# rrwick/Autocycler

Measured on AMD Instinct MI355X. Metric: Mbp/sec through compress->unitig GFA (k=51), higher is better.
Workload: dtype u64

## Files before the change

autocycler_amd/_capi.py:

```python
import ctypes as C
import os
from pathlib import Path

_HERE = Path(__file__).resolve().parent
LIB_PATH = _HERE / "libautocycler_hip.so"


class HipLibraryMissing(RuntimeError):
    pass


class AutocyclerError(RuntimeError):
    """The text the reference would hand to quit_with_error (misc.rs:131-137)."""


class SeqView(C.Structure):
    _fields_ = [("fwd", C.c_char_p), ("length", C.c_uint32), ("id", C.c_uint16)]


class Position(C.Structure):
    _fields_ = [("pos", C.c_uint32), ("seq_id_and_strand", C.c_uint16)]


class Link(C.Structure):
# ... 164 lines not shown
    _fields_ = [("a", C.c_uint16), ("b", C.c_uint16), ("distance", C.c_double)]


class ClusterSummary(C.Structure):
    _fields_ = [("n_seqs", C.c_uint32), ("launches", C.c_uint32), ("rescans", C.c_uint64), ("compares", C.c_uint64), ("seconds", C.c_double)]

    def as_dict(self):
        return {n: getattr(self, n) for n, _ in self._fields_}


class ClusterQcRecord(C.Structure):
    _fields_ = [("node", C.c_uint16), ("container", C.c_uint16), ("size", C.c_uint32), ("assembly_count", C.c_uint32), ("fail", C.c_uint32),
                ("trusted", C.c_uint32), ("reserved", C.c_uint32), ("median_length", C.c_uint64), ("cluster_dist", C.c_double)]

    def as_dict(self):
        return {n: getattr(self, n) for n, _ in self._fields_ if n != "reserved"}


class ClusteringMetrics(C.Structure):
    _fields_ = [(n, C.c_uint32) for n in ("pass_cluster_count", "fail_cluster_count", "pass_contig_count", "fail_contig_count")] + \
               [(n, C.c_double) for n in ("pass_contig_fraction", "fail_contig_fraction", "cluster_balance_score", "cluster_tightness_score",
                                          "overall_clustering_score")]

    def as_dict(self):
        return {n: getattr(self, n) for n, _ in self._fields_}


class ClusterQcSummary(C.Structure):
    _fields_ = [(n, C.c_uint32) for n in ("n_seqs", "n_clusters", "rounds", "evaluations", "pair_batches", "launches", "readbacks", "reserved")] + \
               [(n, C.c_uint64) for n in ("alternatives", "node_pairs", "bytes_read_back")] + [("seconds", C.c_double), ("start_score", C.c_double)]

    def as_dict(self):
        return {n: getattr(self, n) for n, _ in self._fields_ if n != "reserved"}


class DepthGraph(C.Structure):
    _fields_ = [("seq_bytes", C.c_void_p), ("seq_begin", C.c_void_p), ("seq_len", C.c_void_p), ("n_unitigs", C.c_uint32),
                ("links", C.c_void_p), ("n_links", C.c_uint64)]


class DepthTotals(C.Structure):
    _fields_ = [("size", C.c_uint64)] + \
               [(n, C.c_uint64) for n in ("reads", "rejected_reads", "read_bases", "span_bases", "span_kmers", "hits", "distinct_kmers", "repeat_kmers",
                                          "table_slots")] + [("batches", C.c_uint32), ("launches", C.c_uint32), ("seconds_device", C.c_double)]

    def as_dict(self):
        return {n: getattr(self, n) for n, _ in self._fields_ if n != "size"}

ALLREDUCE_FN = C.CFUNCTYPE(C.c_int, C.c_void_p, C.c_void_p, C.c_uint64, C.c_int, C.c_int)

EXPORTS = ["ac_compress_build", "ac_compress_build_multi", "ac_multi_info_get", "ac_compress_build_device", "ac_pack_text", "ac_text_size", "ac_layout_text", "ac_kmer_count",
           "ac_stats_pre", "ac_stats_post", "ac_unitig_count", "ac_unitig", "ac_unitigs_bulk", "ac_paths_bulk", "ac_unitig_positions", "ac_links",
           "ac_path", "ac_timings_get", "ac_timings_get_sized", "ac_free", "ac_gfa_string", "ac_string_free", "ac_last_error",
           "ac_device_count", "ac_max_kmer", "ac_version", "ac_abi_version", "ac_set_host_side_device", "ac_source_hash", "ac_set_stage_timing", "ac_random_access_ceilings", "ac_random_access_ceilings_at", "ac_release_memory", "ac_end_repair_device", "ac_pairwise_distances", "ac_trim_paths", "ac_trim_path_slices", "ac_overlap_alignment", "ac_trim_max_unitigs", "ac_resolve_bridges", "ac_resolve_bridge_paths", "ac_path_distances", "ac_resolve_anchors", "ac_resolve_bridge_records", "ac_resolve_best_paths", "ac_resolve_distinct_paths", "ac_resolve_summary_get_sized", "ac_resolve_max_path", "ac_resolve_free", "ac_graph_components", "ac_components_from_links", "ac_components_records", "ac_components_of_unitig", "ac_components_members", "ac_components_unitig_flags", "ac_components_summary_get_sized", "ac_topology_name", "ac_components_free", "ac_graph_merge_plan", "ac_merge_plan_from_links", "ac_merge_chains", "ac_merge_members", "ac_merge_chain_of_unitig", "ac_merge_fixed_flags", "ac_merge_sequences", "ac_merge_links", "ac_merge_summary_get_sized", "ac_merge_free", "ac_graph_subsets", "ac_subsets_from_paths", "ac_subsets_records", "ac_subsets_unitigs", "ac_subsets_links", "ac_subsets_seqs", "ac_subsets_path_ends", "ac_subsets_dense", "ac_subsets_summary_get_sized", "ac_subsets_free", "ac_subsets_components", "ac_subsets_merge_plan", "ac_subsets_merged_paths", "ac_merged_paths_get", "ac_merged_paths_summary_get_sized", "ac_merged_paths_free", "ac_merge_finish", "ac_subsets_finish", "ac_finished_unitigs", "ac_finished_sequences", "ac_finished_new_of_old", "ac_finished_links", "ac_finished_paths", "ac_finished_summary_get_sized", "ac_finished_free", "ac_finished_gfa_string", "ac_finished_to_graph", "ac_apply_bridges", "ac_graph_resolve_apply", "ac_applied_unitigs", "ac_applied_bridge_of", "ac_applied_links", "ac_applied_bridge_sequences", "ac_applied_summary_get_sized", "ac_applied_free", "ac_applied_merge_plan", "ac_applied_finish", "ac_applied_gfa_string", "ac_resolve_graphs", "ac_clean_graph", "ac_graph_clean", "ac_cleaned_unitigs", "ac_cleaned_links", "ac_cleaned_summary_get_sized", "ac_cleaned_free", "ac_cleaned_merge_plan", "ac_cleaned_finish", "ac_cleaned_gfa_string", "ac_parse_tig_numbers", "ac_gfa_segment_types", "ac_clean_gfa", "ac_clean", "ac_trim_apply", "ac_graph_trim_apply", "ac_graph_trim", "ac_trimmed_records", "ac_trimmed_summary_get_sized", "ac_trimmed_free", "ac_trimmed_subsets", "ac_trimmed_finish", "ac_trimmed_yaml_string", "ac_trim_gfa", "ac_trim_dir", "ac_resolve_dir", "ac_cluster_tree_build", "ac_cluster_tree_from_distances", "ac_cluster_tree_from_nodes", "ac_cluster_nodes", "ac_cluster_merges", "ac_cluster_summary_get_sized", "ac_cluster_free", "ac_cluster_max_seqs", "ac_cluster_cut", "ac_cluster_assign", "ac_cluster_containment", "ac_cluster_newick", "ac_cluster_generate", "ac_cluster_qc_nodes", "ac_cluster_qc_clusters", "ac_cluster_qc_assignment", "ac_cluster_qc_records", "ac_cluster_qc_metrics", "ac_cluster_qc_trace", "ac_cluster_qc_summary_get_sized", "ac_cluster_qc_free", "ac_cluster_min_assemblies", "ac_cluster_seq_inputs", "ac_depth_begin", "ac_depth_begin_handles", "ac_depth_add_reads", "ac_depth_add_fastq", "ac_depth_totals_get", "ac_depth_kmer_counts", "ac_depth_finish", "ac_depth_free", "ac_selftest_primitives", "ac_selftest_scan", "ac_selftest_radix", "ac_selftest_segments", "ac_selftest_sort_cmp", "ac_selftest_scan_pool", "ac_selftest_wave", "ac_selftest_fills", "ac_selftest_fill_order", "ac_selftest_readback", "ac_selftest_scalar_chain", "ac_selftest_arena", "ac_selftest_launch", "ac_selftest_atomics", "ac_selftest_side_order", "ac_selftest_event_ring", "ac_verify_graph", "ac_verify_graph_device", "ac_graph_from_gfa", "ac_graph_kmer_size", "ac_graph_seq_info", "ac_decompress_seq", "ac_decompress_device", "ac_decompress",
           "ac_shard_begin", "ac_shard_fragment_sizes", "ac_shard_fragments_export", "ac_shard_build_union", "ac_shard_fragment_packed_words", "ac_shard_fragments_export_packed", "ac_shard_build_union_packed",
           "ac_shard_unitig_count", "ac_shard_table_capacity", "ac_shard_bitmap_words", "ac_shard_bitmap_export", "ac_shard_build_novel", "ac_shard_sib_words", "ac_shard_sib_export", "ac_shard_degrees",
           "ac_shard_degree_bytes", "ac_multi_info_get_sized", "ac_shard_links_export", "ac_shard_links_import",
           "ac_shard_query_count", "ac_shard_query_key_words", "ac_shard_queries_export", "ac_shard_answer", "ac_shard_walk", "ac_shard_queries_route", "ac_shard_walk_routed", "ac_shard_local_distinct", "ac_shard_set_distinct_upper_bound", "ac_shard_distinct_count", "ac_shard_degrees_export", "ac_shard_build_graph", "ac_gfa_string_parts", "ac_shard_reduce_export", "ac_shard_reduce_import", "ac_shard_finish", "ac_shard_set_allreduce", "ac_device_copy",
           "ac_shard_path_entries", "ac_shard_paths_export", "ac_shard_free", "ac_graph_set_paths", "ac_graph_seq_count", "ac_path_counts",
           "ac_seqs_load", "ac_seqs_from_raw", "ac_seqs_count", "ac_seqs_assembly_count", "ac_seqs_views", "ac_seqs_get",
           "ac_seqs_repair_seconds", "ac_seqs_metrics_yaml", "ac_seqs_free", "ac_compress_seqs", "ac_compress_dir", "ac_compress_dir_multi"]

_libs = {}


def load_library(path=None):
    path = Path(path) if path else LIB_PATH
    key = str(path)
    if key in _libs:
        return _libs[key]
    if not path.exists():
        raise HipLibraryMissing(f"{path} not found: build the HIP extension first (make -C autocycler_amd/csrc). "
                                "There is no CPU fallback.")
    try:
        if os.environ.get("AC_NO_TORCH"):
            raise ImportError
        import torch
    except ImportError:
        pass
    lib = C.CDLL(key)
    lib.ac_last_error.restype = C.c_char_p
    lib.ac_version.restype = C.c_char_p
    lib.ac_source_hash.restype = C.c_char_p
    lib.ac_kmer_count.restype = C.c_uint64
    lib.ac_kmer_count.argtypes = [C.c_void_p]
    lib.ac_stats_pre.restype = Stats
    lib.ac_stats_pre.argtypes = [C.c_void_p]
    lib.ac_stats_post.restype = Stats
    lib.ac_stats_post.argtypes = [C.c_void_p]
    lib.ac_unitig_count.restype = C.c_uint32
    lib.ac_unitig_count.argtypes = [C.c_void_p]
    lib.ac_max_kmer.restype = C.c_uint32
    lib.ac_text_size.restype = C.c_uint64
    lib.ac_free.argtypes = [C.c_void_p]
    lib.ac_string_free.argtypes = [C.c_void_p]
    lib.ac_unitig.argtypes = [C.c_void_p, C.c_uint32, C.POINTER(C.c_void_p), C.POINTER(C.c_uint32), C.POINTER(C.c_double)]
    lib.ac_unitig_positions.argtypes = [C.c_void_p, C.c_uint32, C.c_int, C.POINTER(C.POINTER(Position)), C.POINTER(C.c_uint32)]
    lib.ac_links.argtypes = [C.c_void_p, C.POINTER(C.POINTER(Link)), C.POINTER(C.c_uint64)]
    lib.ac_path.argtypes = [C.c_void_p, C.c_uint32, C.POINTER(C.POINTER(C.c_int32)), C.POINTER(C.c_uint32)]
    lib.ac_timings_get.argtypes = [C.c_void_p, C.POINTER(Timings)]
    lib.ac_shard_unitig_count.restype = C.c_uint32
    lib.ac_shard_unitig_count.argtypes = [C.c_void_p]
    lib.ac_shard_fragment_packed_words.restype = C.c_uint64
    lib.ac_shard_fragment_packed_words.argtypes = [C.c_void_p, C.c_uint64]
    lib.ac_shard_local_distinct.restype = C.c_uint64
    lib.ac_shard_local_distinct.argtypes = [C.c_void_p]
    lib.ac_shard_set_distinct_upper_bound.argtypes = [C.c_void_p, C.c_uint64]
# ... 136 lines not shown
    lib.ac_trimmed_summary_get_sized.argtypes = [C.c_void_p, C.POINTER(TrimmedSummary), C.c_size_t]
    lib.ac_trimmed_free.restype = None
    lib.ac_trimmed_free.argtypes = [C.c_void_p]
    lib.ac_trimmed_subsets.restype = C.c_void_p
    lib.ac_trimmed_subsets.argtypes = [C.c_void_p]
    lib.ac_trimmed_finish.argtypes = [C.c_void_p, C.c_void_p, C.c_void_p, C.c_int, C.POINTER(C.c_void_p)]
    lib.ac_trimmed_yaml_string.argtypes = [C.c_void_p, C.POINTER(C.c_void_p), C.POINTER(C.c_uint64)]
    lib.ac_trim_gfa.argtypes = [C.c_char_p, C.c_uint64, C.c_double, C.c_uint32, C.c_double, C.c_int, C.POINTER(C.c_void_p), C.POINTER(C.c_uint64), C.POINTER(C.c_void_p),
                                C.POINTER(TrimmedSummary)]
    lib.ac_trim_dir.argtypes = [C.c_char_p, C.c_double, C.c_uint32, C.c_double, C.c_int]
    lib.ac_resolve_dir.argtypes = [C.c_char_p, C.c_int]
    lib.ac_resolve_graphs.argtypes = [C.c_void_p, C.c_int, C.POINTER(C.c_void_p), C.POINTER(C.c_void_p), C.POINTER(C.c_void_p), C.POINTER(C.c_uint32)]
    lib.ac_cluster_tree_from_nodes.argtypes = [C.POINTER(ClusterNode), C.c_uint32, C.c_int32, C.POINTER(C.c_void_p)]
    lib.ac_cluster_nodes.argtypes = [C.c_void_p, C.POINTER(C.POINTER(ClusterNode)), C.POINTER(C.c_uint32), C.POINTER(C.c_int32)]
    lib.ac_cluster_merges.argtypes = [C.c_void_p, C.POINTER(C.POINTER(ClusterMerge)), C.POINTER(C.c_uint32)]
    lib.ac_cluster_summary_get_sized.restype = C.c_size_t
    lib.ac_cluster_summary_get_sized.argtypes = [C.c_void_p, C.POINTER(ClusterSummary), C.c_size_t]
    lib.ac_cluster_free.argtypes = [C.c_void_p]
    lib.ac_cluster_free.restype = None
    lib.ac_cluster_cut.argtypes = [C.c_void_p, C.c_double, C.c_void_p, C.c_uint32, C.c_void_p, C.POINTER(C.c_uint32)]
    lib.ac_cluster_assign.argtypes = [C.c_void_p, C.c_void_p, C.c_uint32, C.c_void_p, C.c_void_p, C.c_void_p, C.POINTER(C.c_uint32)]
    lib.ac_cluster_containment.argtypes = [C.c_void_p, C.c_uint32, C.c_void_p, C.c_uint32, C.c_double, C.c_void_p, C.c_void_p]
    lib.ac_cluster_newick.argtypes = [C.c_void_p, C.c_void_p, C.c_int, C.POINTER(C.c_void_p)]
    qc_in = [C.c_void_p, C.c_void_p, C.c_uint32, C.c_void_p, C.c_void_p, C.c_void_p, C.c_void_p, C.c_double, C.c_uint32]
    lib.ac_cluster_generate.argtypes = qc_in + [C.c_void_p, C.c_uint32, C.c_int, C.POINTER(C.c_void_p)]
    lib.ac_cluster_qc_nodes.argtypes = qc_in + [C.c_void_p, C.c_uint32, C.c_void_p, C.c_uint32, C.c_int, C.POINTER(C.c_void_p)]
    lib.ac_cluster_qc_clusters.argtypes = [C.c_void_p, C.POINTER(C.POINTER(C.c_uint16)), C.POINTER(C.c_uint32)]
    lib.ac_cluster_qc_assignment.argtypes = [C.c_void_p, C.POINTER(C.POINTER(C.c_uint16)), C.POINTER(C.c_uint32)]
    lib.ac_cluster_qc_records.argtypes = [C.c_void_p, C.POINTER(C.POINTER(ClusterQcRecord)), C.POINTER(C.c_uint32)]
    lib.ac_cluster_qc_metrics.argtypes = [C.c_void_p, C.POINTER(ClusteringMetrics)]
    lib.ac_cluster_qc_trace.argtypes = [C.c_void_p, C.POINTER(C.POINTER(C.c_uint32)), C.POINTER(C.c_uint32), C.POINTER(C.POINTER(C.c_double)),
                                        C.POINTER(C.POINTER(C.c_uint8)), C.POINTER(C.c_uint64)]
    lib.ac_cluster_qc_summary_get_sized.restype = C.c_size_t
    lib.ac_cluster_qc_summary_get_sized.argtypes = [C.c_void_p, C.POINTER(ClusterQcSummary), C.c_size_t]
    lib.ac_cluster_qc_free.argtypes = [C.c_void_p]
    lib.ac_cluster_qc_free.restype = None
    lib.ac_cluster_min_assemblies.argtypes = [C.c_void_p, C.c_uint32, C.POINTER(C.c_uint32)]
    lib.ac_cluster_seq_inputs.argtypes = [C.c_void_p, C.c_void_p, C.c_void_p, C.c_void_p, C.c_void_p, C.POINTER(C.c_uint32)]
    lib.ac_depth_begin.argtypes = [C.c_uint32, C.POINTER(DepthGraph), C.c_uint32, C.c_int, C.POINTER(C.c_void_p)]
    lib.ac_depth_begin_handles.argtypes = [C.c_uint32, C.POINTER(C.c_void_p), C.c_uint32, C.c_int, C.POINTER(C.c_void_p)]
    lib.ac_depth_add_reads.argtypes = [C.c_void_p, C.c_void_p, C.c_void_p, C.c_uint64]
    lib.ac_depth_add_fastq.argtypes = [C.c_void_p, C.c_char_p]
    lib.ac_depth_totals_get.argtypes = [C.c_void_p, C.POINTER(DepthTotals)]
    lib.ac_depth_kmer_counts.argtypes = [C.c_void_p, C.c_void_p, C.c_uint64, C.c_void_p, C.c_void_p, C.c_void_p]
    lib.ac_depth_finish.argtypes = [C.c_void_p, C.c_uint32, C.c_void_p, C.c_void_p]
    lib.ac_depth_free.argtypes = [C.c_void_p]
    lib.ac_depth_free.restype = None
    lib.ac_selftest_scan.argtypes = [C.c_int, C.c_int, C.c_void_p, C.c_uint64, C.c_int, C.c_int, C.c_int, C.c_void_p]
    lib.ac_selftest_radix.argtypes = [C.c_int, C.c_void_p, C.c_void_p, C.c_uint64, C.c_int, C.c_int, C.c_int, C.c_uint64, C.c_int, C.c_int, C.c_void_p, C.c_void_p]
    lib.ac_selftest_segments.argtypes = [C.c_int, C.c_int, C.c_void_p, C.c_void_p, C.c_uint64, C.c_uint64, C.c_int, C.c_void_p, C.POINTER(C.c_uint32)]
    lib.ac_selftest_sort_cmp.argtypes = [C.c_int, C.c_int, C.c_void_p, C.c_void_p, C.c_void_p, C.c_uint64, C.c_void_p, C.c_void_p, C.c_void_p]
    lib.ac_selftest_scan_pool.argtypes = [C.c_int, C.c_int, C.c_uint64, C.POINTER(C.c_uint64)]
    lib.ac_selftest_wave.argtypes = [C.c_int, C.c_int, C.c_void_p, C.c_void_p, C.c_void_p, C.c_void_p]
    lib.ac_selftest_fills.argtypes = [C.c_int, C.c_void_p, C.c_uint64, C.c_int, C.c_int, C.c_void_p, C.c_uint64, C.c_void_p]
    lib.ac_selftest_fill_order.argtypes = [C.c_int, C.c_uint64, C.c_int, C.c_uint64, C.c_uint64, C.c_int, C.c_uint64, C.c_int, C.c_uint64, C.c_int, C.c_void_p]
    lib.ac_selftest_readback.argtypes = [C.c_int, C.c_void_p, C.c_uint64, C.c_int, C.c_void_p, C.c_uint64, C.c_void_p, C.c_void_p]
    lib.ac_selftest_scalar_chain.argtypes = [C.c_int, C.c_void_p, C.c_uint64, C.c_void_p, C.c_void_p]
    lib.ac_selftest_arena.argtypes = [C.c_int, C.c_void_p, C.c_uint64, C.c_void_p, C.c_void_p, C.c_void_p, C.c_void_p]
    lib.ac_selftest_launch.argtypes = [C.c_int, C.c_int, C.c_uint64, C.c_void_p, C.c_void_p]
    lib.ac_selftest_atomics.argtypes = [C.c_int, C.c_int, C.c_uint64, C.c_uint64, C.c_void_p, C.c_void_p, C.c_uint32, C.c_void_p, C.c_void_p]
    lib.ac_selftest_side_order.argtypes = [C.c_int, C.c_int, C.c_int, C.c_uint32, C.c_uint64, C.c_void_p]
    lib.ac_selftest_event_ring.argtypes = [C.c_int, C.c_int, C.c_void_p, C.c_uint32, C.c_void_p]
    _libs[key] = lib
    return lib


def _check(lib, rc):
    if rc != 0:
        raise AutocyclerError(lib.ac_last_error().decode(errors="replace"))


class Graph:

    def __init__(self, lib, handle, n_seqs):
        self._lib, self._h, self.n_seqs = lib, handle, n_seqs

    def close(self):
        if self._h:
            self._lib.ac_free(self._h)
            self._h = None

    def __del__(self):
        try:
            self.close()
        except Exception:
            pass

    @property
    def kmer_count(self):
        return self._lib.ac_kmer_count(self._h)

    def _stats(self, fn):
        s = fn(self._h)
        return dict(unitigs=s.unitigs, links=s.links_one_way, total_length=s.total_length)

    @property
    def stats_pre(self):
        return self._stats(self._lib.ac_stats_pre)

    @property
    def stats_post(self):
        return self._stats(self._lib.ac_stats_post)

    @property
    def unitig_count(self):
        return self._lib.ac_unitig_count(self._h)

# ... 1476 lines not shown
    v = _np_in(vals, np.int32 if signed else np.uint32)
    ko, vo = np.empty_like(k), np.empty_like(v)
    _check(lib, lib.ac_selftest_radix(device, k.ctypes.data, v.ctypes.data, k.size, begin_bit, end_bit, int(signed), prep_n, prep_bits, int(prep_reuse),
                                      ko.ctypes.data, vo.ctypes.data))
    return ko, vo


def selftest_segments(op, seg, vals, n_segments, deferred_err=False, device=0, lib_path=None):
    import numpy as np
    lib = load_library(lib_path)
    s, v = _np_in(seg, np.uint32), _np_in(vals, np.uint64)
    out = np.empty(n_segments, dtype=np.uint64 if op == "min" else np.uint32)
    err = C.c_uint32()
    _check(lib, lib.ac_selftest_segments(device, {"min": 0, "argmin": 1}[op], s.ctypes.data, v.ctypes.data, s.size, n_segments, int(deferred_err), out.ctypes.data,
                                         C.byref(err)))
    return out, err.value


def selftest_sort_pairs_cmp(key_a, key_b, vals, device=0, lib_path=None):
    import numpy as np
    lib = load_library(lib_path)
    a, b, v = _np_in(key_a, np.uint64), _np_in(key_b, np.uint32), _np_in(vals, np.uint32)
    ao, bo, vo = np.empty_like(a), np.empty_like(b), np.empty_like(v)
    _check(lib, lib.ac_selftest_sort_cmp(device, 0, a.ctypes.data, b.ctypes.data, v.ctypes.data, a.size, ao.ctypes.data, bo.ctypes.data, vo.ctypes.data))
    return ao, bo, vo


def selftest_sort_indices_cmp(values, indices, device=0, lib_path=None):
    import numpy as np
    lib = load_library(lib_path)
    a, v = _np_in(values, np.uint64), _np_in(indices, np.uint32)
    vo = np.empty_like(v)
    _check(lib, lib.ac_selftest_sort_cmp(device, 1, a.ctypes.data, None, v.ctypes.data, v.size, None, None, vo.ctypes.data))
    return vo


def selftest_scan_pool(op="read", value=0, device=0, lib_path=None):
    lib = load_library(lib_path)
    out = (C.c_uint64 * 3)()
    _check(lib, lib.ac_selftest_scan_pool(device, {"read": 0, "advance": 1, "invalidate": 2}[op], value, out))
    return dict(cap=out[0], epoch=out[1], tickets=out[2])


def selftest_wave(program, in_u64, aux_i32, live_mask, out_init, device=0, lib_path=None):
    import numpy as np
    lib = load_library(lib_path)
    i, a, m = _np_in(in_u64, np.uint64), _np_in(aux_i32, np.int32), _np_in(live_mask, np.uint64)
    out = np.array(out_init, dtype=np.uint64)
    assert i.size == 256 and a.size == 256 and m.size == 4 and out.size == 256
    _check(lib, lib.ac_selftest_wave(device, program, i.ctypes.data, a.ctypes.data, m.ctypes.data, out.ctypes.data))
    return out


FILL_KINDS = {"all": 0, "from": 1, "first": 2, "side_stream": 3}
FILL_TRIGGERS = {"none": 0, "launch": 1, "launch_full": 2, "launch_wave_kernel": 3, "copy_h2d": 4, "copy_d2h": 5, "copy_d2d": 6, "stream_sync": 7,
                 "arena_rewind": 8, "after_main": 9, "main_event": 10}
READ_PATHS = {"copy_d2h": 0, "batch": 1, "batch_twice": 2, "to_host": 3, "read_scalar": 4, "side_stream": 5}
ARENA_OPS = {"alloc": 0, "mark": 1, "rewind": 2, "reset": 3, "reserve": 4, "release_all": 5, "set_grow": 6}
LAUNCHERS = {"launch": 0, "launch_full": 1, "launch_wave_kernel": 2, "sized": 3}
ATOMIC_OPS = {"add32": 0, "add64": 1, "min32": 2, "max32": 3, "min64": 4, "max64": 5, "or32": 6, "or64": 7, "xor64": 8, "fetch_or32": 9, "fetch_and32": 10,
              "cas32": 11, "cas64": 12, "load32": 13, "wave_alloc32": 14, "wave_add64": 15}
ATOMIC_THREADS = 64 * 256
LAUNCH_SLOTS = 1024


def selftest_fills(regions, trigger, pattern, drop_on_reset=False, device=0, lib_path=None):
    import numpy as np
    lib = load_library(lib_path)
    r = _np_in([(b, FILL_KINDS[k], a, v) for b, k, a, v in regions], np.uint64)
    span = np.array(pattern, dtype=np.uint8)
    launches = np.zeros(2, dtype=np.uint32)
    _check(lib, lib.ac_selftest_fills(device, r.ctypes.data, len(regions), FILL_TRIGGERS[trigger], int(drop_on_reset), span.ctypes.data, span.size, launches.ctypes.data))
    return span, (int(launches[0]), int(launches[1]))


def selftest_fill_order(n, byte1, w_lo, w_hi, w_val, from2, byte2, upto3, byte3, device=0, lib_path=None):
    import numpy as np
    lib = load_library(lib_path)
    out = np.empty(n, dtype=np.uint8)
    _check(lib, lib.ac_selftest_fill_order(device, n, byte1, w_lo, w_hi, w_val, from2, byte2, upto3, byte3, out.ctypes.data))
    return out


def selftest_readback(data, path, items, device=0, lib_path=None):
    import numpy as np
    lib = load_library(lib_path)
    d = _np_in(data, np.uint8)
    it = _np_in(items, np.uint64).reshape(-1, 2)
    out = np.full(int(it[:, 1].sum()) + 1, 0xA5, dtype=np.uint8)
    counters = np.zeros(2, dtype=np.uint32)
    _check(lib, lib.ac_selftest_readback(device, d.ctypes.data, d.size, READ_PATHS[path], it.ctypes.data, it.shape[0], out.ctypes.data, counters.ctypes.data))
    assert out[-1] == 0xA5
    ends = np.cumsum(it[:, 1]).astype(np.int64)
    return [out[e - int(b):e] for e, b in zip(ends, it[:, 1])], int(counters[0]), int(counters[1])


def selftest_scalar_chain(values, device=0, lib_path=None):
    import numpy as np
    lib = load_library(lib_path)
    v = _np_in(values, np.uint64)
    out = np.zeros_like(v)
    counters = np.zeros(2, dtype=np.uint32)
    _check(lib, lib.ac_selftest_scalar_chain(device, v.ctypes.data, v.size, out.ctypes.data, counters.ctypes.data))
    return out, int(counters[0]), int(counters[1])


# ... 108 lines not shown
```

autocycler_amd/csrc/capi_steps.cpp:

```cpp
#include <algorithm>
#include <cstddef>
#include <cstring>
#include <fstream>
#include <memory>
#include <string>

#include "capi_common.hpp"
#include "gfa_writer.hpp"
#include "graph_depth.hpp"

using namespace ac;
using namespace ac::abi;

extern "C" {

int ac_end_repair_device(uint32_t k, void* d_text, uint64_t n_text, const uint64_t* seq_off, const uint32_t* seq_len,
                         uint16_t* seq_d1, uint16_t* seq_d2, uint32_t n_seqs, int device, double* seconds, uint64_t* n_matches) {
    return guarded([&] {
        if (!d_text || n_seqs == 0) throw DeviceError("no sequences found in input assemblies");
        if (!seq_d1 || !seq_d2) throw DeviceError("null sequence table");
        {
            std::vector<uint16_t> zero(n_seqs, 0);
            validate_layout(k, n_text, seq_off, seq_len, zero.data(), zero.data(), n_seqs);
        }
// ... 1717 lines not shown
        DeviceCall call(device);
        VerifyReport r;
#ifdef AC_EMU
        verify_graph_device(g->g, text.data(), text.size(), off, len, &r);
#else
        void* d_text = nullptr;
        AC_HIP_CHECK(hipMalloc(&d_text, text.size() + 64));
        struct Free { void* p; ~Free() { (void)hipFree(p); } } fr{d_text};
        AC_HIP_CHECK(hipMemcpy(d_text, text.data(), text.size(), hipMemcpyHostToDevice));
        verify_graph_device(g->g, (const uint8_t*)d_text, text.size(), off, len, &r);
#endif
        fill_report(r, report);
    });
}

int ac_decompress_device(const ac_graph* g, int device, uint8_t* out, uint64_t out_bytes) {
    return guarded([&] {
        if (!g || !out) throw DeviceError("null pointer");
        if (!g->host_arrays || !g->host_paths) throw DeviceError("this rank kept no host arrays (sharded build, not the writing rank)");
        uint64_t need = 0;
        for (uint32_t l : g->seq_lens) need += l;
        if (out_bytes < need) throw DeviceError("ac_decompress_device: the buffer holds " + std::to_string(out_bytes) + " bytes, the sequences need " + std::to_string(need));
        DeviceCall call(device);
        decompress_device(g->g, g->seq_lens, out);
    });
}
int ac_selftest_primitives(int device, uint64_t n, uint64_t seed, int end_bit, int key_kind) {
    return guarded([&] {
        if (end_bit < 1 || end_bit > 64) throw DeviceError("end_bit out of range");
        DeviceCall call(device);
        primitives_selftest(n, seed, end_bit, key_kind);
    });
}
int ac_selftest_scan(int device, int kind, const void* in, uint64_t n, int in_place, int misalign_in, int misalign_out, void* out) {
    return guarded([&] { DeviceCall call(device); selftest_scan(kind, in, n, in_place != 0, misalign_in, misalign_out, out); });
}
int ac_selftest_radix(int device, const uint64_t* keys, const void* vals, uint64_t n, int begin_bit, int end_bit, int val_kind, uint64_t prep_n, int prep_bits,
                      int prep_reuse, uint64_t* keys_out, void* vals_out) {
    return guarded([&] { DeviceCall call(device); selftest_radix(keys, vals, n, begin_bit, end_bit, val_kind, prep_n, prep_bits, prep_reuse != 0, keys_out, vals_out); });
}
int ac_selftest_segments(int device, int op, const uint32_t* seg, const uint64_t* vals, uint64_t n, uint64_t n_segments, int deferred_err, void* out, uint32_t* err_out) {
    return guarded([&] { DeviceCall call(device); selftest_segments(op, seg, vals, n, n_segments, deferred_err != 0, out, err_out); });
}
int ac_selftest_sort_cmp(int device, int form, const uint64_t* key_a, const uint32_t* key_b, const uint32_t* vals, uint64_t n, uint64_t* key_a_out, uint32_t* key_b_out,
                         uint32_t* vals_out) {
    return guarded([&] { DeviceCall call(device); selftest_sort_cmp(form, key_a, key_b, vals, n, key_a_out, key_b_out, vals_out); });
}
int ac_selftest_scan_pool(int device, int op, uint64_t value, uint64_t* out) {
    return guarded([&] { DeviceCall call(device); selftest_scan_pool(op, value, out); });
}
int ac_selftest_wave(int device, int program, const uint64_t* in_u64, const int32_t* aux_i32, const uint64_t* live_mask, uint64_t* out_u64) {
    return guarded([&] { DeviceCall call(device); selftest_wave(program, in_u64, aux_i32, live_mask, out_u64); });
}
int ac_selftest_fills(int device, const uint64_t* regions, uint64_t n_regions, int trigger, int mode, uint8_t* span, uint64_t span_bytes, uint32_t* launches_out) {
    return guarded([&] { DeviceCall call(device); selftest_fills(regions, n_regions, trigger, mode, span, span_bytes, launches_out); });
}
int ac_selftest_fill_order(int device, uint64_t n, int byte1, uint64_t w_lo, uint64_t w_hi, int w_val, uint64_t from2, int byte2, uint64_t upto3, int byte3, uint8_t* out) {
    return guarded([&] { DeviceCall call(device); selftest_fill_order(n, byte1, w_lo, w_hi, w_val, from2, byte2, upto3, byte3, out); });
}
int ac_selftest_readback(int device, const uint8_t* data, uint64_t n_data, int path, const uint64_t* items, uint64_t n_items, uint8_t* out, uint32_t* counters_out) {
    return guarded([&] { DeviceCall call(device); selftest_readback(data, n_data, path, items, n_items, out, counters_out); });
}
int ac_selftest_scalar_chain(int device, const uint64_t* values, uint64_t n, uint64_t* out, uint32_t* counters_out) {
    return guarded([&] { DeviceCall call(device); selftest_scalar_chain(values, n, out, counters_out); });
}
int ac_selftest_arena(int device, const uint64_t* ops, uint64_t n_ops, uint64_t* totals_out, uint64_t* allocs_out, const uint8_t* live, uint64_t* wrong_out) {
    return guarded([&] { DeviceCall call(device); selftest_arena(ops, n_ops, totals_out, allocs_out, live, wrong_out); });
}
int ac_selftest_launch(int device, int which, uint64_t n, uint64_t* slots_out, uint32_t* info_out) {
    return guarded([&] { DeviceCall call(device); selftest_launch(which, n, slots_out, info_out); });
}
int ac_selftest_atomics(int device, int op, uint64_t init, uint64_t expected, const uint64_t* operand, const uint32_t* target, uint32_t n_words, uint64_t* words_out,
                        uint64_t* returns_out) {
    return guarded([&] { DeviceCall call(device); selftest_atomics(op, init, expected, operand, target, n_words, words_out, returns_out); });
}
int ac_selftest_side_order(int device, int mode, int which, uint32_t seed, uint64_t n_words, uint32_t* out_words) {
    return guarded([&] { DeviceCall call(device); selftest_side_order(mode, which, seed, n_words, out_words); });
}
int ac_selftest_event_ring(int device, int op, const uint8_t* kinds, uint32_t n_more, uint64_t* out) {
    return guarded([&] { DeviceCall call(device); selftest_event_ring(op, kinds, n_more, out); });
}

int ac_random_access_ceilings_at(int device, uint64_t table_slots, double* cas_gops, double* read_gops) {
    return guarded([&] {
        DeviceCall call(device);
        random_access_ceilings(cas_gops, read_gops, table_slots);
    });
}
int ac_random_access_ceilings(int device, double* cas_gops, double* read_gops) { return ac_random_access_ceilings_at(device, (uint64_t)1 << 24, cas_gops, read_gops); }

}
```

autocycler_amd/csrc/graph_build.hpp:

```cpp
#pragma once
#include <cstdint>
#include <functional>
#include <string>
#include <vector>

#include "graph_types.hpp"
#include "trim_host.hpp"
#include "resolve_host.hpp"
#include "components_host.hpp"
#include "merge_host.hpp"
#include "subset_host.hpp"
#include "trim_apply_host.hpp"
#include "finish_host.hpp"
#include "apply_host.hpp"
#include "clean_host.hpp"
#include "cluster_host.hpp"
#include "cluster_qc_host.hpp"

namespace ac {

struct SeqView {
    const uint8_t* fwd;
    uint32_t length;
};
// ... 125 lines not shown
void path_distance_batch(const PathPool& pool, const std::vector<PathPair>& pairs, const uint32_t* weights, std::vector<uint32_t>* dist,
                         ResolveDeviceStats* st);
uint32_t resolve_max_path();
struct ClusterDeviceStats { double seconds = 0; uint64_t rescans = 0, compares = 0; uint32_t launches = 0; };
void cluster_merges_device(const double* asym, uint32_t n, std::vector<ClusterRowMerge>* merges, ClusterDeviceStats* st);
void cluster_merges_graph_device(const FinalGraph& g, uint32_t n_seqs, double* asym_out, std::vector<ClusterRowMerge>* merges, ClusterDeviceStats* st);
uint32_t cluster_max_seqs();
struct ClusterQcDeviceStats {
    double seconds = 0;
    uint32_t launches = 0, readbacks = 0, evaluations = 0, pair_batches = 0;
    uint64_t alternatives = 0, pairs_counted = 0, bytes_read_back = 0;
};
void cluster_qc_device(const double* asym, uint32_t n, const uint32_t* dfs_tip, double cutoff, const std::function<void(const ClusterQcEvaluate&)>& body,
                       ClusterQcDeviceStats* st);
void components_device(uint32_t n_unitigs, const Link* links, uint64_t n_links, const uint32_t* unitig_len, const uint8_t* alive, const uint8_t* marked,
                       ComponentsResult* out);
struct MergePlanInput {
    uint32_t n_unitigs = 0; const Link* links = nullptr; uint64_t n_links = 0; const uint32_t* unitig_len = nullptr; const uint8_t* alive = nullptr;
    const uint8_t* seed_fixed = nullptr; const int32_t* path = nullptr; uint64_t n_path = 0;
    const uint8_t* seq_bytes = nullptr; const uint64_t* seq_begin = nullptr; uint64_t seq_total = 0;
};
void merge_plan_device(const MergePlanInput& in, MergeResult* out);
struct SubsetInput {
    uint32_t n_unitigs = 0; const Link* links = nullptr; uint64_t n_links = 0; const uint32_t* unitig_len = nullptr; const uint8_t* alive = nullptr;
    const int32_t* path = nullptr; const uint64_t* path_off = nullptr; uint32_t n_clusters = 0; const SubsetPlan* plan = nullptr;
};
void subsets_device(const SubsetInput& in, SubsetResult* out);
struct MergedPathsInput {
    uint32_t n_unitigs = 0; const uint32_t* unitig_len = nullptr; const int32_t* path = nullptr; const uint64_t* path_off = nullptr;
    const SubsetPlan* plan = nullptr; size_t kept_first = 0, kept_count = 0; const MergeResult* merge = nullptr;
};
void merged_paths_device(const MergedPathsInput& in, MergedPathsResult* out);
struct TrimApplyInput {
    uint32_t n_unitigs = 0; const Link* links = nullptr; uint64_t n_links = 0; const uint32_t* unitig_len = nullptr; const uint8_t* alive = nullptr;
    const int32_t* path = nullptr; const uint64_t* path_off = nullptr; double mad = 0;
};
void trim_apply_device(const TrimApplyInput& in, TrimApplyPlan* tp, SubsetPlan* plan, SubsetResult* out);
struct FinishInput {
    uint32_t n_unitigs = 0; const Link* links = nullptr; uint64_t n_links = 0; const uint32_t* unitig_len = nullptr; const uint8_t* alive = nullptr;
    const double* depth = nullptr; const uint8_t* type = nullptr; const uint8_t* seq_bytes = nullptr; const uint64_t* seq_begin = nullptr; uint64_t seq_total = 0;
    const MergeResult* plan = nullptr; const int32_t* path = nullptr; uint64_t n_path = 0; bool renumber = false; uint64_t unitigs_after = 0;
};
void merge_finish_device(const FinishInput& in, FinishResult* out);
void apply_bridges_device(const ApplyInput& in, const ApplyPlan& plan, ApplyResult* out);
void clean_device(const CleanInput& in, CleanResult* out);
void primitives_selftest(uint64_t n, uint64_t seed, int end_bit, int key_kind);
void selftest_scan(int kind, const void* in, uint64_t n, bool in_place, int misalign_in, int misalign_out, void* out);
void selftest_radix(const uint64_t* keys, const void* vals, uint64_t n, int begin_bit, int end_bit, int val_kind, uint64_t prep_n, int prep_bits, bool prep_reuse,
                    uint64_t* keys_out, void* vals_out);
void selftest_segments(int op, const uint32_t* seg, const uint64_t* vals, uint64_t n, uint64_t n_segments, bool deferred_err, void* out, uint32_t* err_out);
void selftest_sort_cmp(int form, const uint64_t* a, const uint32_t* b, const uint32_t* vals, uint64_t n, uint64_t* a_out, uint32_t* b_out, uint32_t* vals_out);
void selftest_scan_pool(int op, uint64_t value, uint64_t* out);
void selftest_wave(int program, const uint64_t* in_u64, const int32_t* aux_i32, const uint64_t* live_mask, uint64_t* out_u64);
void selftest_fills(const uint64_t* regions, uint64_t n_regions, int trigger, int mode, uint8_t* span, uint64_t span_bytes, uint32_t* launches_out);
void selftest_fill_order(uint64_t n, int byte1, uint64_t w_lo, uint64_t w_hi, int w_val, uint64_t from2, int byte2, uint64_t upto3, int byte3, uint8_t* out);
void selftest_readback(const uint8_t* data, uint64_t n_data, int path, const uint64_t* items, uint64_t n_items, uint8_t* out, uint32_t* counters_out);
void selftest_scalar_chain(const uint64_t* values, uint64_t n, uint64_t* out, uint32_t* counters_out);
void selftest_arena(const uint64_t* ops, uint64_t n_ops, uint64_t* totals_out, uint64_t* allocs_out, const uint8_t* live, uint64_t* wrong_out);
void selftest_launch(int which, uint64_t n, uint64_t* slots_out, uint32_t* info_out);
void selftest_atomics(int op, uint64_t init, uint64_t expected, const uint64_t* operand, const uint32_t* target, uint32_t n_words, uint64_t* words_out, uint64_t* returns_out);
void selftest_side_order(int mode, int which, uint32_t seed, uint64_t n_words, uint32_t* out_words);
void selftest_event_ring(int op, const uint8_t* kinds, uint32_t n_more, uint64_t* out);

void random_access_ceilings(double* cas_gops, double* read_gops, uint64_t table_slots = (uint64_t)1 << 24);

void device_warmup(int device, uint32_t k = 0, uint64_t text_bytes_estimate = 0);

void pack_text_host(const uint8_t* text, uint64_t n_text, uint64_t* bits, uint32_t* mask32, bool force_scalar);

void release_host_stager();

int max_supported_k();
void tuning_refresh();
int tuning_multi_transport();
bool tuning_multi_fragments_as_bytes();
bool tuning_multi_tail_replicated();
void set_stage_timing(bool on);
bool stage_timing();

}
```

autocycler_amd/csrc/graph_impl.hpp:

```cpp
#pragma once
#include "graph_build.hpp"

#include <chrono>
#include <cmath>
#include <map>
#include <string>
#include <algorithm>
#include <atomic>
#include <thread>
#include <functional>
#include <condition_variable>
#include <mutex>
#include <fcntl.h>
#include <unistd.h>
#if defined(__x86_64__)
#include <immintrin.h>
#endif

#include "device_rt.hpp"

namespace ac {

static double now_s() {
    return std::chrono::duration<double>(std::chrono::steady_clock::now().time_since_epoch()).count();
// ... 424 lines not shown
        seq_off.alloc(n_seqs); seq_len.alloc(n_seqs); seq_d1.alloc(n_seqs); seq_d2.alloc(n_seqs);
        copy_h2d(seq_off.ptr(), off.data(), (size_t)n_seqs * 8);
        copy_h2d(seq_len.ptr(), len.data(), (size_t)n_seqs * 4);
        copy_h2d(seq_d1.ptr(), d1.data(), (size_t)n_seqs * 2);
        copy_h2d(seq_d2.ptr(), d2.data(), (size_t)n_seqs * 2);
        has_flags = flags != nullptr;
        if (flags) { seq_flags.alloc(n_seqs); copy_h2d(seq_flags.ptr(), flags->data(), n_seqs); }
        n_bases = 0; any_dots = 0; n_dotted = 0; expected_nonbase = (u64)n_seqs + 1;
        for (u32 i = 0; i < n_seqs; i++) { n_bases += len[i]; if (d1[i] || d2[i]) { any_dots = 1; n_dotted++; } expected_nonbase += (u64)d1[i] + d2[i]; }
        stream_sync();
    }
    void alloc_table(u32 n) { n_seqs = n; h_off.clear(); h_len.clear(); seq_off.alloc(n); seq_len.alloc(n); seq_d1.alloc(n); seq_d2.alloc(n); seq_flags.alloc(n); has_flags = true; }
    void set_sums(u64 bases, u64 dotted, u64 dots) { n_bases = bases; n_dotted = dotted; any_dots = dotted ? 1 : 0; expected_nonbase = (u64)n_seqs + 1 + dots; }
    TextCtx ctx(int k) const { return TextCtx{bits.ptr(), mask.ptr(), n_text, k, seq_off.ptr(), seq_len.ptr(), seq_d1.ptr(), seq_d2.ptr(), n_seqs}; }
    bool packed = false;
    void pack_alloc(stream_t s = 0) {
        u64 n_bits_words = n_text / 32 + 24, n_mask_words = n_text / 64 + 12;
        bits.alloc(n_bits_words); mask.alloc(n_mask_words);
        const u64 groups = (n_text + 31) / 32;
        bits.fill_bytes_from(groups * 8, 0, s);
        mask.fill_bytes_from(groups * 4, 0xFF, s);
        if (check_alphabet) { pack_bad.alloc(2); pack_bad.fill_bytes(0xFF, s); }
    }
    void verify_alphabet(const u32* bad) const {
        if (!check_alphabet) return;
        if (bad[0] != 0xFFFFFFFFu) throw DeviceError("input sequence " + std::to_string(index_base + bad[0]) + " contains non-ACGT characters");
        const u64 found = (u64)(u32)(bad[1] + 1u);
        if (found != (expected_nonbase & 0xFFFFFFFFULL))
            throw DeviceError("the text does not match its sequence table: " + std::to_string(expected_nonbase) + " padding dots and separators expected, " +
                              std::to_string(found) + " non-ACGT characters found");
    }
    void pack() {
        if (packed) return;
        pack_alloc();
        launch((n_text + 31) / 32, PackFunctor{d_text, n_text, bits.ptr(), (u32*)mask.ptr(), 0, chk()});
        packed = true;
    }
};

struct GraphBuilder::Impl {
    u32 k = 0;
    DBuf<u8> text_owned;
    PackedText loc;
    PackedText uni;
    PackedText* G = &loc;
    BuildTimings* tm = nullptr;
    double t0 = 0, t_begin = 0;
    void lap(double* acc) { if (!g_stage_timing) return; stream_sync(); double t = now_s(); *acc += t - t0; t0 = t; }

    DBuf<u32> counters;
    DBuf<u64> slots; u64 cap = 0; u64 N = 0;
    DBuf<u64> bm; DBuf<u32> wprefix; DBuf<u64> npos;
    u32 U = 0;
    DBuf<u32> kinfo, head, scan, ustart, order, rank, ulen;
    DBuf<u64> ustartpos, useq_off; DBuf<u8> uorient;
    DBuf<int32_t> links; DBuf<u64> wlinks;
    DBuf<u32> depth, minpos_fwd, minpos_rev; DBuf<u64> path_off; DBuf<int32_t> ent_val; u64 n_ent = 0;
    DBuf<u64> wl_text; DBuf<u32> depth_u, minpos_fwd_u, minpos_rev_u, run_start, run_end;
    void walk_arrays();
    void walk_tables(bool filter);
    void walk_to_seed_order();
    bool walked_plain = false;
    DBuf<u8> fs0, fe0;
    u32 pos_cap_now = 0xFFFFFFFFu; bool exact_positions = false;
    bool host_remap_allowed = false;
    bool paths_in_seed_numbers = false;
    bool checked_sorts = false; DBuf<u32> sort_flags;
    bool deferred_sort_checks() const { return host_remap_allowed_build && !checked_sorts && sort_checks_deferrable(); }
    bool host_remap_allowed_build = false;
    DBuf<u8> maybe_dest; bool maybe_dest_valid = false;
    DBuf<u8> frag_text; DBuf<u64> frag_meta, frag_fpos, frag_boff; u64 frag_bytes = 0, n_frags = 0;
    u64 distinct_upper = 0;

    void begin(BuildTimings* t) {
        tm = t; t_begin = t0 = now_s();
        rt_counters() = RtCounters();
        host_remap_allowed = false;
        counters.alloc(8); counters.fill_bytes(0);
        sort_flags.alloc(2); sort_flags.fill_bytes(0);
    }
    void check_sizes(const PackedText& t) const {
        if (t.n_text >= POS_MASK) throw DeviceError("input too large for 40-bit text positions");
        if (t.n_seqs == 0 || t.n_text < (u64)k + 2) throw DeviceError("no sequences");
    }
    template <int W> void insert(const PackedText& t, u32 hint, DBuf<u64>* slots_out, u64* cap_out, u64* n_distinct_out, DBuf<u64>* bm_out, bool want_sib = false);
    DBuf<u64> sflags;
    DBuf<u64> runs; DBuf<u32> run_count; u64 run_rows = 0, run_rows_cap = 0;
    DBuf<u64> loc_bm; DBuf<u32> loc_wprefix; bool local_insert_of_shard = false;
    struct CopyPlan { bool ok = false; u64 R = 0, NW = 0, Rb = 0; DBuf<RunRec> rr; DBuf<u32> rseq; DBuf<u64> wfirst, w_begin, w_end; DBuf<u32> w_gap; } cplan;
    void occupancy_bitmap(const DBuf<u64>& sl, u64 c, DBuf<u64>* occ_out, const u64* sflags_in, u64* sib_out, stream_t s = 0);
    DBuf<u64> occ;
    DBuf<u64> sib;
    DBuf<u64> sibn; bool sib_pending = false;
    DBuf<u32> kcontrib, pend, pidx; u64 n_pending = 0, n_first = 0;
    DBuf<u64> endset, endset_bloom; u64 endset_mask = 0;
    u32 n_owners = 1, my_owner = 0;
    void* upload_done = nullptr; u64 upload_avail = 0; bool upload_pending = false;
    struct UploadJob {
#ifndef AC_EMU
        const std::vector<SeqView>* seqs = nullptr;
        std::vector<uint64_t> off;
        uint32_t k = 0; u64 n = 0, CH = 0, SUB = 0, n_chunks = 0, slot_bytes = 0; int NSLOT = 0, dev = 0;
        hipStream_t up = nullptr, pk = nullptr;
        u64* d_bits = nullptr;
        bool direct = false;
        double t_start = 0; std::atomic<u64> chunks_issued{0}; std::atomic<double> t_last{0};
        hipEvent_t fills_done = nullptr;
// ... 13 lines not shown
    void finish_upload();
    ~Impl();
    void pack_overlapped(u32 hint) {
        PackedText& pt = loc;
        if (pt.packed) return;
#ifndef AC_EMU
        const u64 p_end_all = pt.n_text - (u64)k + 1;
        const u64 first = std::max<u64>(p_end_all / std::max<u32>(hint, 1), 1u << 16);
        const u64 H = (first + (u64)k + 8192 + 4095) & ~4095ULL;
        const u64 cap_est = next_pow2(std::max<u64>(1024, pt.n_bases / std::max<u32>(hint, 1) * 3 + 4096));
        if (cap_est <= (1ULL << 25) && H + (1u << 22) < pt.n_text) {
            pt.pack_alloc();
            launch(H / 32, PackFunctor{pt.d_text, pt.n_text, pt.bits.ptr(), (u32*)pt.mask.ptr(), 0, pt.chk()});
            SideStream& side = SideStream::get();
            side.after_main();
            launch((pt.n_text + 31) / 32 - H / 32, PackFunctor{pt.d_text, pt.n_text, pt.bits.ptr(), (u32*)pt.mask.ptr(), H / 32, pt.chk()}, side.stream());
            upload_done = side.mark(); upload_avail = H; upload_pending = true;
            pt.packed = true;
            return;
        }
#endif
        pt.pack();
    }
    Table graph_table() const { return Table{const_cast<u64*>(slots.ptr()), cap - 1, occ.ptr(), nullptr, n_owners, my_owner, nullptr, nullptr, nullptr, nullptr, 0}; }
    template <int W> void fragments();
    template <int W> void table();
    void novel_list(u64 known_n);
    template <int W> void degrees();
    template <int W> void walk_queries();
    template <int W> void answer_queries(const u64* d_keys, u64 n, u64* d_out);
    DBuf<u64> qkeys; u64 n_queries = 0;
    DBuf<u32> qidx;
    DBuf<u64> qanswers;
    template <int W> void route_queries(u32 n_shards, u64* d_routed_keys, u64* counts_host);
    const u64* walk_answers = nullptr;
    template <int W> void unitigs();
    template <int W> void walk();
    template <int W> bool walk_copy_prepare(u32 PC, const Novel& nv_text);
    template <int W> void walk_copy_finish(u32 PC);
    void tail(FinalGraph* out, bool want_graph, bool want_paths);
    std::function<void(void*, uint64_t, int, int)> tail_xchg;
};

inline void GraphBuilder::Impl::occupancy_bitmap(const DBuf<u64>& sl, u64 c, DBuf<u64>* occ_out, const u64* sflags_in, u64* sib_out, stream_t s) {
    occ_out->alloc((c + 63) / 64);
#ifdef AC_EMU
    occ_out->fill_bytes(0);
#endif
    launch_full(c, MarkFunctor{sl.ptr(), occ_out->ptr(), sflags_in, sib_out}, s);
}
inline void GraphBuilder::Impl::novel_list(u64 known_n) {
    PackedText& g = *G;
    u64 n_bm_words = g.n_text / 64 + 1;
    DBuf<u32> wcnt(n_bm_words + 1);
    wprefix.alloc(n_bm_words + 1);
    launch(n_bm_words + 1, PopcFunctor{bm.ptr(), wcnt.ptr(), n_bm_words});
    exclusive_scan_u32(wcnt.ptr(), wprefix.ptr(), n_bm_words + 1);
    if (known_n) N = known_n;
    else {
        N = read_scalar(wprefix.ptr() + n_bm_words);
        if (N == 0) throw DeviceError("internal error: no k-mers in the union of the shards");
        tm->n_distinct = N;
    }
    npos.alloc(N);
    launch_wave_kernel(fill_novel_wave_kernel<0>, (n_bm_words + 255) / 256, 0, (const u64*)bm.ptr(), (const u32*)wprefix.ptr(), npos.ptr(), n_bm_words);
    kinfo.alloc(N, true);
    head.alloc(N + 1); scan.alloc(N + 1);
    head.fill_bytes_from(N * 4, 0); scan.fill_bytes_from(N * 4, 0);
    lap(&tm->collect_sort);
}

inline void GraphBuilder::Impl::walk_arrays() {
    wl_text.alloc((u64)U * 10);
    depth_u.alloc(U, true); minpos_fwd_u.alloc(U); minpos_rev_u.alloc(U);
    run_start.alloc((u64)U + 1, true); run_end.alloc((u64)U + 1, true);
}
inline void GraphBuilder::Impl::walk_tables(bool filter) {
    launch((u64)U * 10, WlinkFlagFunctor{filter ? maybe_dest.ptr() : nullptr, wlinks.ptr(), counters.ptr() + 4});
    const u32 pos_init = pos_cap_now == 0xFFFFFFFFu ? 0xFFFFFFFFu : ((pos_cap_now + 1) | POS_BOUND);
    launch((u64)U * 10, WlinkTextOrderFunctor{wlinks.ptr(), rank.ptr(), order.ptr(), uorient.ptr(), wl_text.ptr(), minpos_fwd_u.ptr(), minpos_rev_u.ptr(), pos_init});
}
inline void GraphBuilder::Impl::walk_to_seed_order() {
    depth.alloc(U); minpos_fwd.alloc(U); minpos_rev.alloc(U);
    DBuf<u32> started, ended;
    if (walked_plain) {
        started.alloc((u64)U + 1); ended.alloc((u64)U + 1);
        inclusive_scan_u32(run_start.ptr(), started.ptr(), (u64)U + 1);
        exclusive_scan_u32(run_end.ptr(), ended.ptr(), (u64)U + 1);
    }
    launch(U, WalkToSeedOrderFunctor{order.ptr(), depth_u.ptr(), walked_plain ? started.ptr() : nullptr, walked_plain ? ended.ptr() : nullptr,
                                     minpos_fwd_u.ptr(), minpos_rev_u.ptr(), depth.ptr(), minpos_fwd.ptr(), minpos_rev.ptr()});
}

template <int W> struct Stages {
    static void table(GraphBuilder::Impl& m);
    static void degrees(GraphBuilder::Impl& m);
    static void walk_queries(GraphBuilder::Impl& m);
    static void answer_queries(GraphBuilder::Impl& m, const u64* d_keys, u64 n, u64* d_out);
    static void route_queries(GraphBuilder::Impl& m, u32 n_shards, u64* d_routed_keys, u64* counts_host);
    static void unitigs(GraphBuilder::Impl& m);
    static void walk(GraphBuilder::Impl& m);
    static void fragments(GraphBuilder::Impl& m);
    static void warm();
};

void tail_warm();

#define AC_DISPATCH_W(NAME, ARGS)                                        \
    switch (key_words((int)impl_->k)) {                                  \
        case 1: Stages<1>::NAME ARGS; break;                             \
        case 2: Stages<2>::NAME ARGS; break;                             \
        case 3: Stages<3>::NAME ARGS; break;                             \
        case 4: Stages<4>::NAME ARGS; break;                             \
        case 8: Stages<8>::NAME ARGS; break;                             \
        case 16: Stages<16>::NAME ARGS; break;                           \
        default: throw DeviceError("unsupported k");                     \
    }

}
```

autocycler_amd/csrc/graph_stages.hip:

```cpp
#include "graph_impl.hpp"

namespace ac {

template <int W>
void GraphBuilder::Impl::insert(const PackedText& pt, u32 hint, DBuf<u64>* slots_out, u64* cap_out, u64* n_distinct_out, DBuf<u64>* bm_out, bool want_sib) {
    TextCtx t = pt.ctx((int)k);
    const u64 p_end_all = pt.n_text - (u64)k + 1;
    if (hint == 0) hint = 1;
    u64 est = pt.n_bases / hint;
    u64 c = next_pow2(std::max<u64>(1024, est * 3 + 4096));
    if (&pt == &uni && distinct_upper) {
        const u64 mine = distinct_upper / std::max<u32>(n_owners, 1) + distinct_upper / (8 * (u64)std::max<u32>(n_owners, 1)) + 4096;
        c = next_pow2(std::max<u64>(1024, mine * 10 / 7));
    }
    if (c > next_pow2(pt.n_bases * 2 + 1024)) c = next_pow2(pt.n_bases * 2 + 1024);
    const int shift = table_shift() >= 0 ? table_shift() : (c > (1ULL << 25) ? 0 : 1);
    c <<= shift;
    struct CapMemo { u64 n_text = 0, cap = 0; u32 k = 0; int shift = -2; u32 owners = 0; };
    static thread_local CapMemo memo[4]; static thread_local unsigned memo_next = 0;
    const u32 memo_owners = (&pt == &uni) ? n_owners : 1u;
    for (const CapMemo& m : memo)
        if (pt.n_text == m.n_text && k == m.k && m.shift == table_shift() && m.owners == memo_owners && m.cap > c) c = m.cap;
    const int copy_mode = (&pt == &loc && (want_sib || (local_insert_of_shard && shard_path_copy()))) ? path_copy() : 0;
    bool want_runs = false;
// ... 269 lines not shown
            { ReadBatch rb; rb.add(&hp[0], pidx.ptr() + N, 4); rb.add(&hp[1], fslot.ptr() + g.n_seqs, 4); rb.run(); }
            n_pending = hp[0]; n_first = hp[1];
            kc_tmp.alloc(n_pending + n_first + 1); kc_tmp.fill_bytes(0);
            kout = kc_tmp.ptr();
        }
        launch((u64)DEG_LISTS * DEG_REGIONS * DEG_PROBE_THREADS, DegreeProbeFunctor<W>{g.ctx((int)k), tb, npos.ptr(), kout, g.any_dots, wk, es, by_index ? pidx.ptr() : nullptr});
#ifdef AC_EMU
        if (knobs().degree_diag) {
            u64 c0 = 0, c1 = 0;
            for (u32 r = 0; r <= DEG_REGIONS; r++) { c0 += wk.count(0)[r]; c1 += wk.count(1)[r]; }
            fprintf(stderr, "degree diag: N %llu, queued real %llu, generic %llu, left open %llu, any_dots %d\n", (unsigned long long)N,
                    (unsigned long long)c0, (unsigned long long)c1, (unsigned long long)n_pending, (int)g.any_dots);
        }
#endif
        if (by_index) launch(g.n_seqs, FirstFunctor<W>{g.ctx((int)k), tb, nv, kinfo.ptr(), fflags, fslot.ptr(), kc_tmp.ptr() + n_pending});
        items = DBuf<u64>(); counts = DBuf<u32>();
        const u32* kc_src = kc_tmp.ptr();
        kc_tmp = DBuf<u32>();
        Arena::device().rewind(deg_mark);
        if (by_index) {
            kcontrib.alloc(n_pending + n_first + 1);
            const u64 kc_bytes = (n_pending + n_first + 1) * 4;
            if (kcontrib.ptr() != kc_src) {
                const u8* dst_b = (const u8*)kcontrib.ptr(); const u8* src_b = (const u8*)kc_src;
                if (dst_b + kc_bytes <= src_b || src_b + kc_bytes <= dst_b) { Arena::keep_readable(kc_src, kc_bytes); copy_d2d(kcontrib.ptr(), kc_src, kc_bytes); }
                else {
                    const Arena::Mark bounce_mark = Arena::device().mark();
                    DBuf<u32> pad((u64)(src_b + kc_bytes - dst_b) / 4 + 1), bounce(n_pending + n_first + 1);
                    Arena::keep_readable(kc_src, kc_bytes);
                    copy_d2d(bounce.ptr(), kc_src, kc_bytes);
                    copy_d2d(kcontrib.ptr(), bounce.ptr(), kc_bytes);
                    stream_sync();
                    pad = DBuf<u32>(); bounce = DBuf<u32>();
                    Arena::device().rewind(bounce_mark);
                }
            }
            tm->n_degrees_open = n_pending;
            lap(&tm->degree);
            return;
        }
    } else {
        fill_end_set();
        launch(N, DegreeFunctor<W>{g.ctx((int)k), tb, npos.ptr(), kinfo.ptr(), g.any_dots, 0, bm.ptr(), sib.size() && n_owners <= 1 ? sib.ptr() : nullptr, es});
    }
    launch(g.n_seqs, FirstFunctor<W>{g.ctx((int)k), tb, nv, kout, fflags, nullptr, nullptr});
    lap(&tm->degree);
}

template <int W> void GraphBuilder::Impl::unitigs() {
    PackedText& g = *G;
    TextCtx t = g.ctx((int)k);
    Table tb = graph_table();
    Novel nv{bm.ptr(), wprefix.ptr()};
    launch(N, HeadFunctor{npos.ptr(), kinfo.ptr(), head.ptr(), N});
    inclusive_scan_u32(head.ptr(), scan.ptr(), N);
    U = read_scalar(scan.ptr() + (N - 1));
    ustart.alloc((u64)U + 1);
    int seed_keep = seed_prefix_bits();
    if (seed_keep <= 0) { int lg = 1; while ((1ULL << lg) < (u64)U) lg++; seed_keep = std::min(64, ((2 * lg + 8 + 7) / 8) * 8); }
    RadixScratch seed_rs; DBuf<u32> seed_big(1, true);
    if (seed_prefix_sort()) seed_rs.prepare(U, seed_keep);
    launch(N, UnitigStartFunctor{head.ptr(), scan.ptr(), ustart.ptr(), N});
    lap(&tm->segment);

    DBuf<MinVal<W>> umin(U);
    const int mk = minkey_variant() >= 0 ? minkey_variant() : ((W > 4 || (W >= 3 && N >= 32 * (u64)U)) ? 2 : 1);
    if (mk == 2) {
        const u64 n_waves = (N + 63) / 64;
        DBuf<MinPre> upre(U), wfirst(n_waves), wlast(n_waves);
        MinPreArgs a{t, npos.ptr(), scan.ptr(), N, upre.ptr(), wfirst.ptr(), wlast.ptr(), minkey_prefix_bases()};
        launch_wave_kernel(minpre_wave_kernel<W>, (N + 255) / 256, 0, a);
        launch(U, MinFinishFunctor<W>{t, npos.ptr(), ustart.ptr(), U, N, upre.ptr(), wfirst.ptr(), wlast.ptr(), umin.ptr()});
    } else if constexpr (W <= 4) {
        if (mk == 1) {
            const u64 n_waves = (N + 63) / 64;
            DBuf<MinVal<W>> wfirst(n_waves), wlast(n_waves);
            MinWaveArgs<W> a{t, npos.ptr(), scan.ptr(), N, umin.ptr(), wfirst.ptr(), wlast.ptr()};
            launch_wave_kernel(minkey_wave_kernel<W>, (N + 255) / 256, 0, a);
            launch(U, MinJoinFunctor<W>{ustart.ptr(), U, N, wfirst.ptr(), wlast.ptr(), umin.ptr()});
        } else {
            DBuf<MinVal<W>> vals(N); DBuf<u32> seg(N);
            launch(N, CKeyFunctor<W>{t, npos.ptr(), scan.ptr(), vals.ptr(), seg.ptr()});
            reduce_by_segment(seg.ptr(), vals.ptr(), N, umin.ptr(), U, MinOp<W>(), counters.ptr() + 3);
        }
    } else {
        DBuf<u32> umin_idx(U);
        segment_argmin(scan.ptr(), N, umin_idx.ptr(), U, MinIdxOp<W>{t, npos.ptr()}, counters.ptr() + 3);
        launch(U, UnitigMinFunctor<W>{t, npos.ptr(), umin_idx.ptr(), umin.ptr()});
    }
    lap(&tm->minkey);

    order.alloc(U);
    bool seeds_ordered = false;
    if (seed_prefix_sort()) {
        DBuf<u64> wkey(U);
        const int keep = seed_keep;
        DBuf<u32> by_prefix(U);
        launch(U, SeedPrefixFunctor<W>{umin.ptr(), (int)k, wkey.ptr(), keep, by_prefix.ptr()});
        sort_pairs_u64_u32(wkey, by_prefix, U, 64, 0, 64 - keep, &seed_rs);
        DBuf<u32> settled(U); DBuf<u32>& big = seed_big;
        const bool defer = deferred_sort_checks();
        launch(U, SeedTieFunctor<W>{by_prefix.ptr(), wkey.ptr(), U, umin.ptr(), settled.ptr(), seed_max_group(), defer ? sort_flags.ptr() : big.ptr()});
        if (defer || read_scalar(big.ptr()) == 0) {
            order = std::move(settled);
            DBuf<MinVal<W>> sorted(U);
            launch(U, GatherMinFunctor<W>{order.ptr(), umin.ptr(), sorted.ptr()});
            umin = std::move(sorted);
            seeds_ordered = true;
        }
    }
    if (!seeds_ordered) launch(U, IotaFunctor{order.ptr()});
    if (seeds_ordered) {
    } else if constexpr (W <= 4) {
        if ((u64)U >= seed_radix_limit() || seed_prefix_sort()) {
            DBuf<u64> wkey(U);
            for (int word = W - 1; word >= 0; word--) {
                launch(U, MinWordFunctor<W>{order.ptr(), umin.ptr(), word, wkey.ptr()});
                sort_pairs_u64_u32(wkey, order, U, 64);
            }
            DBuf<MinVal<W>> sorted(U);
            launch(U, GatherMinFunctor<W>{order.ptr(), umin.ptr(), sorted.ptr()});
            umin = std::move(sorted);
        } else {
            sort_by_key_cmp(umin, order, U, MinValLess<W>());
        }
    } else {
        sort_keys_cmp(order, U, MinValIdxLess<W>{umin.ptr()});
        DBuf<MinVal<W>> sorted(U);
        launch(U, GatherMinFunctor<W>{order.ptr(), umin.ptr(), sorted.ptr()});
        umin = std::move(sorted);
    }
    rank.alloc(U); ulen.alloc(U); ustartpos.alloc(U); useq_off.alloc((u64)U + 1); uorient.alloc(U);
    DBuf<u64> ulen64((u64)U + 1);
    launch((u64)U + 1, UnitigMetaFunctor<W>{order.ptr(), ustart.ptr(), npos.ptr(), umin.ptr(), U, N, rank.ptr(), ulen.ptr(),
                                            ulen64.ptr(), ustartpos.ptr(), uorient.ptr()});
    exclusive_scan_u64(ulen64.ptr(), useq_off.ptr(), (u64)U + 1);
    UnitigCtx uc{head.ptr(), scan.ptr(), rank.ptr(), uorient.ptr(), ustart.ptr(), ulen.ptr(), U, N};
    lap(&tm->rank);

    links.alloc((u64)U * 10); wlinks.alloc((u64)U * 10);
    DBuf<V16> ui(U);
    launch(U, WalkInfoFunctor{uc, nullptr, ui.ptr()});
    launch((u64)U * 2, LinksFunctor<W>{t, tb, nv, uc, order.ptr(), npos.ptr(), g.any_dots, links.ptr(), wlinks.ptr(), counters.ptr() + 3, ui.ptr()});
    lap(&tm->links);
}

template <int W> void GraphBuilder::Impl::walk_queries() {
    const u32 PC = path_chunk(N, U);
    u64 n_walkers = (loc.n_text + PC - 1) / PC;
    cplan = CopyPlan();
    if (run_rows && loc_bm.size() && PC <= 65535) {
        const u64 nw = loc.n_text / 64 + 1;
        DBuf<u32> wcnt(nw + 1);
        loc_wprefix.alloc(nw + 1);
        launch(nw + 1, PopcFunctor{loc_bm.ptr(), wcnt.ptr(), nw});
        exclusive_scan_u32(wcnt.ptr(), loc_wprefix.ptr(), nw + 1);
        if (walk_copy_prepare<W>(PC, Novel{loc_bm.ptr(), loc_wprefix.ptr()})) n_walkers = cplan.NW;
    }
    n_queries = n_walkers + loc.n_seqs;
    qkeys.alloc(n_queries * W);
    launch(n_queries, WalkQueryFunctor<W>{loc.ctx((int)k), PC, n_walkers, qkeys.ptr(), cplan.ok ? cplan.w_begin.ptr() : nullptr});
}
template <int W> void GraphBuilder::Impl::route_queries(u32 n_shards, u64* d_routed_keys, u64* counts_host) {
    DBuf<u64> owner64(n_queries), first(n_shards);
    qidx.alloc(n_queries);
    first.fill_bytes(0xFF);
    launch(n_queries, QueryOwnerFunctor<W>{qkeys.ptr(), (int)k, n_shards, my_owner, owner64.ptr(), qidx.ptr()});
    int bits = 1;
    while ((1u << bits) < n_shards) bits++;
    sort_pairs_u64_u32(owner64, qidx, n_queries, bits);
    launch(n_queries, OwnerBoundsFunctor{owner64.ptr(), first.ptr()});
    launch(n_queries, QueryGatherFunctor<W>{qkeys.ptr(), qidx.ptr(), d_routed_keys});
    std::vector<u64> h_first = to_host(first, n_shards);
    u64 end = n_queries;
    for (u32 o = n_shards; o-- > 0;) {
        if (h_first[o] == ~0ULL) { counts_host[o] = 0; continue; }
        counts_host[o] = end - h_first[o];
        end = h_first[o];
    }
}
template <int W> void GraphBuilder::Impl::answer_queries(const u64* d_keys, u64 n, u64* d_out) {
    launch(n, AnswerFunctor<W>{G->ctx((int)k), graph_table(), d_keys, d_out});
}

template <int W> bool GraphBuilder::Impl::walk_copy_prepare(u32 PC, const Novel& nv_text) {
    TextCtx t = loc.ctx((int)k);
    cplan = CopyPlan();
    const Arena::Mark mk = Arena::device().mark();
    DBuf<u32> rfirst(run_rows + 1);
    exclusive_scan_u32(run_count.ptr(), rfirst.ptr(), run_rows + 1);
    const u64 R0 = read_scalar(rfirst.ptr() + run_rows);
    if (R0 == 0 || R0 >= 0xFFFFFFF0ULL) { Arena::device().rewind(mk); return false; }
    DBuf<RunRec> sorted(R0);
    launch(run_rows * RUN_ROW, RunGatherFunctor{runs.ptr(), run_count.ptr(), rfirst.ptr(), sorted.ptr()});
    DBuf<u32> ok(R0 + 1), at(R0 + 1); DBuf<u64> covered(1, true); DBuf<u32> overlap(1, true);
    ok.fill_bytes(0);
    DBuf<RunRec> fixed(R0); DBuf<u32> fseq(R0);
    launch(R0, RunFilterFunctor{sorted.ptr(), fixed.ptr(), R0, nv_text, loc.n_text, ok.ptr(), covered.ptr(), t, overlap.ptr(), run_piece(), fseq.ptr()});
    exclusive_scan_u32(ok.ptr(), at.ptr(), R0 + 1);
    const u64 Rb = R0 + loc.n_text / run_piece() + 1;
    CopyPlan& c = cplan;
    c.rr.alloc(Rb); c.rseq.alloc(Rb);
    launch(R0, RunCompactFunctor{fixed.ptr(), ok.ptr(), at.ptr(), c.rr.ptr(), run_piece(), fseq.ptr(), c.rseq.ptr(), nv_text, loc.n_text});
    DBuf<u64> gw(Rb + 2);
    c.wfirst.alloc(Rb + 2);
    launch(Rb + 2, GapWalkersFunctor{c.rr.ptr(), at.ptr() + R0, loc.n_text, PC, gw.ptr()});
    exclusive_scan_u64(gw.ptr(), c.wfirst.ptr(), Rb + 2);
    u64 h_cov = 0, NW = 0; u32 h_R = 0, h_overlap = 0;
    { ReadBatch rb; rb.add(&h_cov, covered.ptr(), 8); rb.add(&h_R, at.ptr() + R0, 4); rb.add(&h_overlap, overlap.ptr(), 4); rb.add(&NW, c.wfirst.ptr() + (Rb + 1), 8); rb.run(); }
    const u64 R = h_R;
    if (knobs().debug_arena) fprintf(stderr, "path copy: %llu runs on the list, %llu pieces usable, covering %llu of %llu positions, %llu walkers\n", (unsigned long long)R0, (unsigned long long)R, (unsigned long long)h_cov, (unsigned long long)loc.n_text, (unsigned long long)NW);
    if (R == 0 || h_overlap || h_cov * 2 < loc.n_text || NW == 0 || NW >= 0xFFFFFFF0ULL) {
        cplan = CopyPlan();
        Arena::device().rewind(mk);
        return false;
    }
    c.w_begin.alloc(NW); c.w_end.alloc(NW); c.w_gap.alloc(NW);
    launch(NW, WalkerRangeFunctor{c.rr.ptr(), R, loc.n_text, PC, c.wfirst.ptr(), c.w_begin.ptr(), c.w_end.ptr(), c.w_gap.ptr()});
    c.R = R; c.NW = NW; c.Rb = Rb; c.ok = true;
    return true;
}
template <int W> void GraphBuilder::Impl::walk_copy_finish(u32 PC) {
    TextCtx t = loc.ctx((int)k), g = G->ctx((int)k);
    Table tb = graph_table();
    Novel nv{bm.ptr(), wprefix.ptr()};
    UnitigCtx uc{head.ptr(), scan.ptr(), rank.ptr(), uorient.ptr(), ustart.ptr(), ulen.ptr(), U, N};
    CopyPlan& c = cplan;
    const u64 R = c.R, NW = c.NW;
    DBuf<u64> wcount(NW + 1), woff(NW + 1);
    const u64 n_slots = ((NW + 63) / 64) * 64 * PC;
    DBuf<int32_t> stage(n_slots); DBuf<u16> stage_off(n_slots);
    DBuf<u32> seq_tid(loc.n_seqs), seq_j(loc.n_seqs);
    wcount.fill_bytes(0);
    const bool filter = maybe_dest_valid;
    walk_tables(filter);
    walked_plain = false;
    DBuf<V16> uinfo(U);
    launch(U, WalkInfoFunctor{uc, filter ? maybe_dest.ptr() : nullptr, uinfo.ptr()});
    launch(NW, PathWalkFunctor<W>{t, g, tb, nv, uc, uinfo.ptr(), wl_text.ptr(), PC, stage.ptr(), wcount.ptr(), seq_tid.ptr(), seq_j.ptr(),
                                 depth_u.ptr(), minpos_fwd_u.ptr(), minpos_rev_u.ptr(), counters.ptr() + 4, filter ? maybe_dest.ptr() : nullptr,
                                 pos_cap_now, 0, walk_answers, NW, c.w_begin.ptr(), c.w_end.ptr(), stage_off.ptr(), nullptr, nullptr});
    exclusive_scan_u64(wcount.ptr(), woff.ptr(), NW + 1);
    const u64 NE = read_scalar(woff.ptr() + NW);
    DBuf<int32_t> ent(NE); DBuf<u64> ent_pos(NE), ent_end(NE); DBuf<u8> ent_want(NE); DBuf<u32> ent_gap(NE);
    launch_full(NW, WalkCompactFunctor{stage.ptr(), stage_off.ptr(), wcount.ptr(), woff.ptr(), c.w_begin.ptr(), c.w_gap.ptr(), PC, NW, uinfo.ptr(),
                                       ent.ptr(), ent_pos.ptr(), ent_end.ptr(), ent_want.ptr(), ent_gap.ptr()});
    DBuf<u64> ra(R), rcnt(R + 1), seg(2 * R + 2), segoff(2 * R + 2); DBuf<u32> cov(NE + 1), copies(NE + 1);
    cov.fill_bytes(0);
    launch(R, RunRangeFunctor{c.rr.ptr(), ent_pos.ptr(), ent_end.ptr(), NE, ra.ptr(), rcnt.ptr(), cov.ptr()});
    launch(2 * R + 2, SegCountFunctor{c.wfirst.ptr(), woff.ptr(), rcnt.ptr(), R, seg.ptr()});
    exclusive_scan_u64(seg.ptr(), segoff.ptr(), 2 * R + 2);
    inclusive_scan_u32(cov.ptr(), copies.ptr(), NE + 1);
    n_ent = read_scalar(segoff.ptr() + (2 * R + 1));
    if (knobs().debug_arena) {
        std::vector<u64> h = to_host(rcnt, R); u64 mx = 0, sum = 0, big = 0, hist[8] = {0};
        for (u64 v : h) { mx = std::max(mx, v); sum += v; if (v > 256) big++; int b = 0; while ((32ull << b) < v && b < 7) b++; hist[b]++; }
        fprintf(stderr, "path copy: %llu pieces, entries per piece: max %llu, mean %.1f, %llu above 256; hist(<=32,64,128,..): %llu %llu %llu %llu %llu %llu %llu %llu\n", (unsigned long long)R, (unsigned long long)mx, (double)sum / (double)R, (unsigned long long)big,
                (unsigned long long)hist[0], (unsigned long long)hist[1], (unsigned long long)hist[2], (unsigned long long)hist[3], (unsigned long long)hist[4], (unsigned long long)hist[5], (unsigned long long)hist[6], (unsigned long long)hist[7]);
    }
    ent_val.alloc(n_ent);
    int32_t* const out_ptr = ent_val.ptr();
    launch(NE, GapOutFunctor{ent.ptr(), ent_gap.ptr(), woff.ptr(), c.wfirst.ptr(), segoff.ptr(), copies.ptr(), out_ptr, depth_u.ptr()});
    launch_full(R * 32, RunOutFunctor<32, 1>{c.rr.ptr(), R, ra.ptr(), rcnt.ptr(), segoff.ptr(), ent.ptr(), ent_pos.ptr(), ent_end.ptr(), uinfo.ptr(),
                                             ent_want.ptr(), t, c.rseq.ptr(), minpos_fwd_u.ptr(), minpos_rev_u.ptr(), out_ptr, pos_cap_now});
    launch(loc.n_seqs, PathOffCopyFunctor{seq_tid.ptr(), seq_j.ptr(), woff.ptr(), c.wfirst.ptr(), c.w_gap.ptr(), segoff.ptr(), path_off.ptr()});
    tm->n_path_entries = n_ent;
    tm->path_runs_copied = R; tm->path_entries_walked = NE;
    copy_h2d(path_off.ptr() + loc.n_seqs, &n_ent, 8);
    launch(loc.n_seqs, PathEndsFunctor{ent_val.ptr(), path_off.ptr(), fs0.ptr(), fe0.ptr(), rank.ptr(), uorient.ptr()});
    walk_to_seed_order();
}

template <int W> void GraphBuilder::Impl::walk() {
    TextCtx t = loc.ctx((int)k), g = G->ctx((int)k);
    Table tb = graph_table();
    Novel nv{bm.ptr(), wprefix.ptr()};
    UnitigCtx uc{head.ptr(), scan.ptr(), rank.ptr(), uorient.ptr(), ustart.ptr(), ulen.ptr(), U, N};
    const u32 PC = path_chunk(N, U);
    u64 n_walkers = (loc.n_text + PC - 1) / PC;
    pos_cap_now = (exact_positions || walk_answers || n_owners > 1 || G != &loc || pos_cap() == 0) ? 0xFFFFFFFFu : pos_cap();
    path_off.alloc((u64)loc.n_seqs + 1);
    const bool filter = path_filter();
    maybe_dest_valid = filter;
    fs0.alloc(U, true); fe0.alloc(U, true);
    walk_arrays();
    DBuf<u64> wcount_plain(n_walkers + 1);
    wcount_plain.fill_bytes(0);
    if (filter) { maybe_dest.alloc((u64)U * 2); launch((u64)U * 2, MaybeDestFunctor{links.ptr(), maybe_dest.ptr()}); }
    if (walk_answers) {
        if (cplan.ok) { walk_copy_finish<W>(PC); lap(&tm->paths); return; }
    } else if (run_rows && n_owners <= 1 && G == &loc && PC <= 65535 && walk_copy_prepare<W>(PC, nv)) { walk_copy_finish<W>(PC); lap(&tm->paths); return; }
    walk_tables(filter);
    walked_plain = true;
    const Arena::Mark walk_mark = Arena::device().mark();
    DBuf<int32_t> stage(((n_walkers + 63) / 64) * 64 * PC);
    DBuf<u64>& wcount = wcount_plain; DBuf<u64> woff(n_walkers + 1);
    DBuf<u32> seq_tid(loc.n_seqs), seq_j(loc.n_seqs);
    DBuf<V16> uinfo(U);
    launch(U, WalkInfoFunctor{uc, filter ? maybe_dest.ptr() : nullptr, uinfo.ptr()});
    launch(n_walkers, PathWalkFunctor<W>{t, g, tb, nv, uc, uinfo.ptr(), wl_text.ptr(), PC, stage.ptr(), wcount.ptr(), seq_tid.ptr(), seq_j.ptr(),
                                        depth_u.ptr(), minpos_fwd_u.ptr(), minpos_rev_u.ptr(), counters.ptr() + 4, filter ? maybe_dest.ptr() : nullptr,
                                        pos_cap_now, path_diag(), walk_answers, n_walkers, nullptr, nullptr, nullptr, run_start.ptr(), run_end.ptr()});
    exclusive_scan_u64(wcount.ptr(), woff.ptr(), n_walkers + 1);
    n_ent = read_scalar(woff.ptr() + n_walkers);
    launch(loc.n_seqs, PathOffFunctor{seq_tid.ptr(), seq_j.ptr(), woff.ptr(), path_off.ptr()});
    tm->n_path_entries = n_ent;
    copy_h2d(path_off.ptr() + loc.n_seqs, &n_ent, 8);
    {
        DBuf<int32_t> packed(n_ent);
        launch_full(((n_walkers + 63) / 64) * 64, PathCompactFunctor{stage.ptr(), wcount.ptr(), woff.ptr(), PC, n_walkers, packed.ptr()});
        const size_t stage_bytes = stage.bytes();
        stage = DBuf<int32_t>(); woff = DBuf<u64>(); seq_tid = DBuf<u32>(); seq_j = DBuf<u32>(); uinfo = DBuf<V16>();
        Arena::device().rewind(walk_mark);
        ent_val.alloc(n_ent);
        const char* const ev = (const char*)ent_val.ptr(); const char* const pk = (const char*)packed.ptr();
        if (n_ent * 4 > stage_bytes || (ev != pk && ev < pk + n_ent * 4 && pk < ev + n_ent * 4))
            throw DeviceError("path walk: the compacted entries overlap the place they are copied to");
        Arena::keep_readable(packed.ptr(), n_ent * 4);
        if (ent_val.ptr() != packed.ptr()) copy_d2d(ent_val.ptr(), packed.ptr(), n_ent * 4);
    }
    launch(loc.n_seqs, PathEndsFunctor{ent_val.ptr(), path_off.ptr(), fs0.ptr(), fe0.ptr(), rank.ptr(), uorient.ptr()});
    walk_to_seed_order();
    lap(&tm->paths);
}

template <int W> void Stages<W>::table(GraphBuilder::Impl& m) { m.template table<W>(); }
template <int W> void Stages<W>::degrees(GraphBuilder::Impl& m) { m.template degrees<W>(); }
template <int W> void Stages<W>::walk_queries(GraphBuilder::Impl& m) { m.template walk_queries<W>(); }
template <int W> void Stages<W>::answer_queries(GraphBuilder::Impl& m, const u64* d_keys, u64 n, u64* d_out) { m.template answer_queries<W>(d_keys, n, d_out); }
template <int W> void Stages<W>::route_queries(GraphBuilder::Impl& m, u32 n_shards, u64* d_routed_keys, u64* counts_host) { m.template route_queries<W>(n_shards, d_routed_keys, counts_host); }
// ... 18 lines not shown
```

autocycler_amd/csrc/graph_tail.hip:

```cpp
#include "graph_impl.hpp"

namespace ac {

[[maybe_unused]] static bool renum_two_pass() { return knobs().renum_two_pass; }
[[maybe_unused]] static u32 renum_max_group() { return knobs().renum_max_group; }
[[maybe_unused]] static void renumber_sort(DBuf<u32>& order, u32 U, const u32* len, const u64* off, const u8* seq, const u32* depth, u32* flag, bool deferred = false,
                                           RadixScratch* sc = nullptr, int len_bits = 32, bool order_is_identity = false) {
    if (U <= 1) return;
    DBuf<u32> backup(deferred && !renum_two_pass() ? 0 : U);
    if (backup.size()) copy_d2d(backup.ptr(), order.ptr(), (size_t)U * 4);
    DBuf<u64> prefix(U), key(U);
    UnitigLess less{len, off, seq, depth};
    u32 zero = 0;
    if (!renum_two_pass()) {
        if (order_is_identity) launch(U, RenumKeyPassFunctor{RenumKeyFunctor{len, off, seq, prefix.ptr()}, RenumPassFunctor{order.ptr(), len, depth, prefix.ptr(), 2, key.ptr()}});
        else {
            launch(U, RenumKeyFunctor{len, off, seq, prefix.ptr()});
            launch(U, RenumPassFunctor{order.ptr(), len, depth, prefix.ptr(), 2, key.ptr()});
        }
        sort_pairs_u64_u32(key, order, U, 32 + std::min(std::max(len_bits, 1), 32), 0, 0, sc);
        launch(U, RenumTieFunctor{order.ptr(), U, len, depth, prefix.ptr(), less, flag, 0, renum_max_group()});
#ifdef AC_EMU
        if (knobs().degree_diag) {
            u64 groups = 0, members = 0, biggest = 0, cur = 1, longest = 0;
// ... 407 lines not shown
        copy_d2d(order2.ptr(), order1.ptr(), (size_t)U * 4);
        renumber_sort(order2, U, clen.ptr(), coff.ptr(), cur, m.depth.ptr(), defer_sorts ? m.sort_flags.ptr() + 1 : renum_flag.ptr(), defer_sorts, &sort2, len_bits);
        number_len.alloc(U); number_len_text.alloc(U); loff.alloc((u64)U + 1);
        number_only.alloc(host_numbers ? U : 0);
        meta.alloc((size_t)U * 24);
        u64* d_seq_begin = (u64*)meta.ptr();
        double* d_depth = (double*)(meta.ptr() + (size_t)U * 8);
        u32* d_seq_len = (u32*)(meta.ptr() + (size_t)U * 16);
        u32* d_seed_index = (u32*)(meta.ptr() + (size_t)U * 20);
        out->k = m.k;
        out->n_kmers = 2 * (u64)m.N;
        out->n_unitigs = U;
        late_by_host = late_copies() == 2 || (late_copies() == 1 && final_total + (u64)U * 28 + n_links * sizeof(Link) >= ((u64)256 << 20));
        launch(U, FinalMetaFunctor{order2.ptr(), coff.ptr(), clen.ptr(), m.depth.ptr(), lcnt.ptr(), number_len.ptr(), d_seq_begin, d_depth,
                                   d_seq_len, lcount.ptr(), host_numbers ? number_only.ptr() : nullptr, d_seed_index, m.order.ptr(), number_len_text.ptr(), m.uorient.ptr()});
        if (host_numbers) {
            number_block = PinnedPool::get().alloc((size_t)U * 4);
            remap_job.path = (int32_t*)out->path_block.p; remap_job.n_ent = m.n_ent;
            if (host_stretch) { remap_job.rec_val = (const int32_t*)rec_val_block.p; remap_job.rec_pos = (const u32*)rec_pos_block.p; remap_job.n_rec = n_stretch; }
            remap_job.number = (const u32*)number_block.p; remap_job.n_unitigs = U;
            remap_job.ent_limit = host_stretch ? (u64)stretch_split_wave * remap_block() : ~0ULL;
            const u32* d_number_only = number_only.ptr();
            const int remap_threads = (int)(host_stretch ? 2 * upload_threads() : upload_threads());
            late_copy([this, U, d_number_only, remap_threads]() {
                copy_d2h_async(number_block.p, d_number_only, (size_t)U * 4, side.stream());
                remap_job.landed = side.mark(); remap_job.side = &side;
#ifndef AC_EMU
                AC_HIP_CHECK(hipGetDevice(&remap_job.dev));
                path_remap_start(remap_job, remap_threads);
#endif
            });
        }
        if (want_graph) {
            out->meta_block = PinnedPool::get().alloc((size_t)U * 24);
            const u8* d_meta = meta.ptr();
            late_copy([this, U, d_meta]() { copy_d2h_async(out->meta_block.p, d_meta, (size_t)U * 24, side.stream()); });
        }
        exclusive_scan_u64(lcount.ptr(), loff.ptr(), (u64)U + 1);
        links_out.alloc(n_links);
        launch(U, LinkOutFunctor{order2.ptr(), L, number_len.ptr(), loff.ptr(), links_out.ptr()});
        if (want_graph) {
            out->links_block = PinnedPool::get().alloc(n_links * sizeof(Link));
            const Link* d_links_out = links_out.ptr();
            late_copy([this, d_links_out]() { copy_d2h_async(out->links_block.p, d_links_out, n_links * sizeof(Link), side.stream()); });
        }
    }

    void finalise_paths() {
        const u64 n_ent = m.n_ent;
        if (host_numbers) {
            const u64 RB = remap_block();
            const u64 n_waves = (n_ent + RB - 1) / RB;
            const u64 w_split = host_stretch ? std::min<u64>(stretch_split_wave, n_waves) : n_waves;
            if (w_split) launch_full(w_split * 64, RemapFunctor{m.ent_val.ptr(), number_len_text.ptr(), m.path_off.ptr(), n_seqs, n_ent, sums.ptr(), 0, (u32)RB, nullptr, false});
            if (w_split < n_waves) {
                const u64 n_chunks = 4, per_chunk = std::max<u64>((n_waves - w_split + n_chunks - 1) / n_chunks, 64);
                for (u64 w = w_split; w < n_waves; w += per_chunk) {
                    const u64 cnt = std::min<u64>(per_chunk, n_waves - w);
                    launch_full(cnt * 64, RemapFunctor{m.ent_val.ptr(), number_len_text.ptr(), m.path_off.ptr(), n_seqs, n_ent, sums.ptr(), w, (u32)RB, nullptr, true});
                    const u64 b = w * RB, e2 = std::min<u64>((w + cnt) * RB, n_ent);
                    const int32_t* d_ent = m.ent_val.ptr();
                    late_copy([this, d_ent, b, e2]() { copy_d2h_async((int32_t*)out->path_block.p + b, d_ent + b, (e2 - b) * 4, side.stream()); });
                }
            }
        } else {
            if (want_paths) out->path_block = PinnedPool::get().alloc(n_ent * 4);
            const u64 RB = remap_block();
            const u64 n_waves = (n_ent + RB - 1) / RB;
            const u64 n_chunks = n_ent * 4 >= ((u64)256 << 20) ? 8 : 4;
            const u64 per_chunk = std::max<u64>((n_waves + n_chunks - 1) / n_chunks, 64);
            int turn = 0;
            for (u64 w = 0; w < n_waves; w += per_chunk) {
                u64 cnt = std::min<u64>(per_chunk, n_waves - w);
                launch_full(cnt * 64, RemapFunctor{m.ent_val.ptr(), number_len_text.ptr(), m.path_off.ptr(), n_seqs, n_ent, sums.ptr(), w, (u32)RB, nullptr, true});
                if (want_paths) {
                    u64 b = w * RB, e2 = std::min<u64>((w + cnt) * RB, n_ent);
                    const int which = n_chunks == 8 ? (turn++ & 1) : 0;
                    side.after_main(which);
                    copy_d2h_async((int32_t*)out->path_block.p + b, m.ent_val.ptr() + b, (e2 - b) * 4, side.stream(which));
                }
            }
        }
        issue_late_copies();
        m.lap(&m.tm->finalize);
    }

    void collect_and_check() {
        const u32 U = m.U; const u64 n_ent = m.n_ent;
        PackedText& loc = m.loc;
        std::vector<u64> h_sums(n_seqs);
        out->path_off.resize((size_t)n_seqs + 1);
        std::vector<u32> errs(8);
        u32 pack_bad[2] = {0xFFFFFFFFu, 0xFFFFFFFFu};
        u32 h_sort_flags[2] = {0, 0};
        u64 n_links_check = 0, final_total_read = 0; u32 h_seq_bad = 0;
        {
            ReadBatch rb;
            rb.add(h_sums.data(), sums.ptr(), (size_t)n_seqs * 8);
            rb.add(out->path_off.data(), m.path_off.ptr(), ((size_t)n_seqs + 1) * 8);
            rb.add(errs.data(), m.counters.ptr(), 8 * 4);
            rb.add(h_sort_flags, m.sort_flags.ptr(), 8);
            rb.add(&n_links_check, loff.ptr() + U, 8);
            if (final_total_pending) rb.add(&final_total_read, noff.ptr() + U, 8);
            if (loc.check_alphabet && loc.pack_bad.size()) rb.add(pack_bad, loc.pack_bad.ptr(), 8);
            if (seq_as_codes) rb.add(&h_seq_bad, seq_bad.ptr(), 4);
            rb.run();
        }
// ... 87 lines not shown
```

autocycler_amd/csrc/kernels_paths.inc:

```
AC_HD u32 idx_of(int32_t v) { return (u32)(v < 0 ? -v : v) - 1; }
struct MaybeDestFunctor {
    const int32_t* links; u8* maybe;
    AC_HD static u64 row(int32_t v) { return ((u64)((u32)(v < 0 ? -v : v) - 1) * 2 + (v > 0 ? 0 : 1)) * 5; }
    AC_HD void operator()(u64 idx) const {
        const u32 x = (u32)(idx >> 1);
        const bool inputs = (idx & 1) == 0;
        const int32_t xnum = (int32_t)x + 1;
        const u64 mine = row(inputs ? -xnum : xnum);
        u32 n = 0;
        bool ok = true;
        for (int c = 0; c < 5; c++) {
            int32_t p = links[mine + (u64)c];
            if (p == 0) continue;
            n++;
            int32_t other = inputs ? -p : p;
            const u64 theirs = row(inputs ? other : -other);
            u32 m = 0; int32_t only = 0;
            for (int d = 0; d < 5; d++) { int32_t q = links[theirs + (u64)d]; if (q != 0) { m++; only = q; } }
            if (!(m == 1 && only == (inputs ? xnum : -xnum))) ok = false;
            if ((u32)(other < 0 ? -other : other) - 1 == x) ok = false;
        }
        maybe[idx] = (ok && n >= 2) ? 1 : 0;
    }
};
// ... 69 lines not shown
        if (!w.live) return;
        if (w.lo == w.hi) atomic_add32(&depth[w.lo], 1u);
        else { atomic_add32(&run_start[w.lo], 1u); atomic_add32(&run_end[w.hi], 1u); }
        w.live = false;
    }
    AC_D void emit(u64 tid, u32& j, u32 f, u32 s_len, u32 r, u32 n, bool strand, u32 want, u64 p, u64 p0, WalkRun& run) const {
        const u64 slot = ((tid >> 6) * (u64)pc + j) * 64 + (tid & 63);
        stage[slot] = strand ? (int32_t)(r + 1) : -(int32_t)(r + 1);
        if (stage_off) stage_off[slot] = (u16)(p - p0);
        j++;
        if ((diag & 3) == 3) return;
        if (!(diag & 1) && !stage_off) {
            if (run.live && r == run.hi + 1) run.hi = r;
            else if (run.live && r + 1 == run.lo) run.lo = r;
            else { run_flush(run); run.lo = run.hi = r; run.live = true; }
        }
        if ((diag & 2) || !want) return;
        u32 other = s_len - n - f;
        if (f > cap && other > cap) return;
        const bool canon = strand == ((uinfo[r].d & 1u) != 0);
        u32 vf = canon ? f : other, vr = canon ? other : f;
        if ((want & 1u) && vf <= cap && vf < minpos_fwd[r]) atomic_min32(&minpos_fwd[r], vf);
        if ((want & 2u) && vr <= cap && vr < minpos_rev[r]) atomic_min32(&minpos_rev[r], vr);
    }
    AC_D void operator()(u64 tid) const {
        const int k = t.k;
        u64 p0 = w_begin ? w_begin[tid] : tid * (u64)pc;
        u32 j = 0;
        WalkRun run{0, 0, false};
        if (p0 >= t.n_text) { cnt[tid] = 0; return; }
        u64 p1 = w_begin ? w_end[tid] : p0 + (u64)pc;
        if (p1 > t.n_text) p1 = t.n_text;
        u32 lo = 0, hi = t.n_seqs;
        while (lo < hi) { u32 mid = lo + ((hi - lo) >> 1); if (t.seq_off[mid] + (u64)t.seq_len[mid] <= p0) lo = mid + 1; else hi = mid; }
        u32 s = lo;
        u64 p = p0;
        while (s < t.n_seqs) {
            u64 s_begin = t.seq_off[s], s_end = s_begin + (u64)t.seq_len[s];
            if (p < s_begin) p = s_begin;
            if (p >= p1) break;
            if (p == s_begin) { seq_tid[s] = (u32)tid; seq_j[s] = j; }
            XKmer<W> x;
            u64 pos; bool rel_same;
            xkmer_in_seq<W>(t, s, p, &x);
            if (ans) {
                const u64 a = ans[p == s_begin ? n_walkers + (u64)s : tid];
                if (!(a >> 63)) { atomic_or32(err, 8u); break; }
                bool flipped;
                (void)xk_canonical<W>(x, k, &flipped);
                pos = a & POS_MASK;
                rel_same = (((a >> 62) & 1) != 0) == flipped;
            } else if (!find_xk<W>(g, tb, x, &pos, &rel_same)) { atomic_or32(err, 8u); break; }
            u32 jn = novel_rank(nv, pos);
            u32 r = uc.scan[jn] - 1;
            const V16 ui = uinfo[r];
            const u32 a = ui.a, b = ui.b;
            bool strand = rel_same;
            const bool at_head = rel_same ? (jn == a) : (jn == b - 1);
            if (at_head) emit(tid, j, (u32)(p - s_begin), (u32)(s_end - s_begin), r, b - a, strand, ui.d >> 1, p, p0, run);
            p += rel_same ? (u64)(b - jn) : (u64)(jn - a + 1);
            bool bad = false;
            u64 cw = ~0ULL, cbits = 0, mw = ~0ULL, mbits = 0;
            while (p < s_end && p < p1) {
                u64 e = p + (u64)k - 1;
                if ((e >> 6) != mw) { mw = e >> 6; mbits = t.mask[mw]; }
                if ((e >> 5) != cw) { cw = e >> 5; cbits = t.bits[cw]; }
                u32 c = ((mbits >> (e & 63)) & 1ULL) ? 4u : (u32)(cbits >> (62 - 2 * (int)(e & 31))) & 3u;
                u64 wl = wlinks[((u64)r * 2 + (strand ? 0 : 1)) * 5 + c];
                int32_t val = (int32_t)(u32)wl;
                if (val == 0) { atomic_or32(err, 16u); bad = true; break; }
                strand = val > 0;
                r = (u32)(strand ? val : -val) - 1;
                const u32 hi = (u32)(wl >> 32);
                emit(tid, j, (u32)(p - s_begin), (u32)(s_end - s_begin), r, hi & WL_LEN_MASK, strand, hi >> 30, p, p0, run);
                p += (u64)(hi & WL_LEN_MASK);
            }
            if (bad) break;
            if (p >= s_end) s++; else break;
        }
        run_flush(run);
        cnt[tid] = j;
    }
};
struct PathCompactFunctor {
    const int32_t* stage; const u64* cnt; const u64* woff; u32 pc; u64 n_walkers; int32_t* ent_val;
    AC_D void operator()(u64 tid, bool valid) const {
        (void)valid;
        const int lane = wv::lane();
        const u64 w0 = tid - (u64)lane;
        if (w0 >= n_walkers) return;
        const bool live = tid < n_walkers;
        const u64 base = woff[w0];
        const u32 rel = live ? (u32)(woff[tid] - base) : 0xFFFFFFFFu;
        const u64 last = (w0 + 63 < n_walkers) ? w0 + 63 : n_walkers - 1;
        const u32 total = (u32)(woff[last] + cnt[last] - base);
        const int32_t* rows = stage + (tid >> 6) * (u64)pc * 64;
        for (u32 o0 = 0; o0 < total; o0 += 64) {
            const u32 o = o0 + (u32)lane;
            int lo = 0;
#pragma unroll
            for (int step = 32; step; step >>= 1) {
                const int cand = lo + step;
                const u32 v = (u32)wv::shfl((int)rel, cand & 63);
                if (cand < 64 && v <= o) lo = cand;
            }
            const u32 start = (u32)wv::shfl((int)rel, lo);
            if (o < total) ent_val[base + o] = rows[(u64)(o - start) * 64 + (u64)lo];
// ... 281 lines not shown
```

autocycler_amd/csrc/kernels_table.inc:

```
struct PackCheck { const u64* seq_off; const u32* seq_len; const u16* d1; const u16* d2; u32 n_seqs; int k; u32* bad; };
AC_D void pack_check(const PackCheck& c, const u8* buf, u64 base, u32 m, u64 n_text) {
    u32 cnt = 0;
    for (u32 mm = m; mm; mm &= mm - 1) {
        const int i = ctz32(mm);
        const u64 p = base + (u64)i;
        if (p >= n_text) break;
        cnt++;
        const u8 ch = buf[i];
        if (c.n_seqs == 0 || p < c.seq_off[0]) { if (!(p == 0 && ch == '$')) atomic_min32(c.bad, 1u); continue; }
        u32 lo = 0, hi = c.n_seqs;
        while (hi - lo > 1) { const u32 mid = lo + ((hi - lo) >> 1); if (c.seq_off[mid] <= p) lo = mid; else hi = mid; }
        const u64 rel = p - c.seq_off[lo], plen = (u64)c.seq_len[lo] + (u64)c.k - 1;
        const bool ok = rel < plen ? (ch == '.' && (rel < c.d1[lo] || rel >= plen - c.d2[lo])) : (rel == plen && ch == '$');
        if (!ok) atomic_min32(c.bad, lo + 1);
    }
    if (cnt) atomic_add32(c.bad + 1, cnt);
}
struct PackFunctor {
    const u8* text; u64 n_text; u64* bits; u32* mask32; u64 first;
    PackCheck chk;
    AC_D void operator()(u64 tid) const {
        tid += first;
        u64 base = tid * 32;
        u64 w = 0; u32 m = 0;
// ... 148 lines not shown
            const int jl = 63 - clz64(hits);
            const u64 qj = (u64)wv::shfl64((unsigned long long)q, jl);
            const bool sj = wv::shfl((int)same, jl) != 0;
            const u64 pj = p + (u64)jl;
            bool again;
            const u64 n = wave_follow(t, pj, qj, sj, c1, lane, tb.runs ? tb.novel : nullptr, &again, p_begin);
            if (PROF) { cy_follow += (u64)clock64() - t0; n_follow++; }
            if (lane == 0) run_note(tb, wave, noted, pj, qj, sj, n);
            if (pj + 1 + n > next) next = pj + 1 + n;
            opener = n >= LONG_RUN || (again && pj + 1 + n >= p + 64);
        }
        p = next;
    }
    if (PROF && lane == 0) {
        atomic_add64(prof + 0, cy_open); atomic_add64(prof + 1, n_open); atomic_add64(prof + 2, cy_wide); atomic_add64(prof + 3, n_wide);
        atomic_add64(prof + 4, cy_follow); atomic_add64(prof + 5, n_follow); atomic_add64(prof + 6, (u64)clock64() - t_wave); atomic_add64(prof + 7, 1);
        atomic_max64(prof + 8, (u64)clock64() - t_wave);
    }
    for (int o = 32; o; o >>= 1) { real += (u32)wv::shfl_xor((int)real, o); claimed += (u32)wv::shfl_xor((int)claimed, o); }
    if (lane == 0) {
        InsertStats* st = stats + (wave & 255);
        atomic_add64(&st->real, (u64)real);
        if (claimed) atomic_add64(&st->claimed, (u64)claimed);
        run_note_done(tb, wave, noted);
    }
}
template <int W> struct RestProbeFunctor {
    TextCtx t; Table tb; u64 pb, pe, stride; u32* out;
    AC_D void operator()(u64 i) const {
        const u64 p = pb + i * stride + (((i + 1) * 0x9E3779B97F4A7C15ULL >> 24) % (stride ? stride : 1));
        if (p >= pe || text_mask_count(t.mask, p, t.k) != 0) return;
        Key<W> fwd = text_extract<W>(t.bits, p, t.k);
        Key<W> rc = key_rc<W>(fwd, t.k);
        Key<W> uk = key_lt<W>(rc, fwd) ? rc : fwd;
        uk.w[0] |= (u64)255 << 56;
        if (!table_owns(tb, key_place<W>(uk, t.k, false, key_hash<W>(uk)).home)) return;
        atomic_add32(out, 1u);
        if (table_find<W>(t, tb, uk, false).found) atomic_add32(out + 1, 1u);
    }
};
struct MarkFunctor {
    const u64* slots; u64* occ; const u64* sflags; u64* sib;
    AC_D void operator()(u64 s, bool valid) const {
        u64 v = valid ? slots[s] : SLOT_EMPTY;
        bool full = v != SLOT_EMPTY;
        u64 b = wv::ballot(full);
        if ((s & 63) == 0 && valid) occ[s >> 6] = b;
        if (!sflags || !full) return;
        const u64 fl = (sflags[s >> 5] >> (2 * (s & 31))) & 3;
        const u64 p = slot_pos(v);
        if (fl) atomic_or64(&sib[p >> 5], fl << (2 * (p & 31)));
    }
};
struct PopcFunctor {
    const u64* bm; u32* cnt; u64 n;
    AC_HD void operator()(u64 w) const { cnt[w] = w < n ? (u32)popc64(bm[w]) : 0u; }
};
template <int UNUSED> AC_KERNEL void __launch_bounds__(256) fill_novel_wave_kernel(const u64* bm, const u32* wprefix, u64* npos, u64 n_words) {
    const u64 w = (u64)wv::bid() * 256 + wv::tid();
    const int lane = wv::lane();
    const u64 w0 = w - (u64)lane;
    if (w0 >= n_words) return;
    const u64 x = w < n_words ? bm[w] : 0;
    const u32 start = w < n_words ? wprefix[w] : 0;
    const u32 cnt = (u32)popc64(x);
    const u32 base = (u32)wv::shfl((int)start, 0);
    const u32 rel = w < n_words ? start - base : 0xFFFFFFFFu;
    const u64 lastv = n_words - w0 - 1;
    const u32 total = (u32)wv::shfl((int)(rel + cnt), lastv > 63 ? 63 : (int)lastv);
    const u32 xlo = (u32)x, xhi = (u32)(x >> 32);
    for (u32 t0 = 0; t0 < total; t0 += 64) {
        const u32 t = t0 + (u32)lane;
        int lo = 0;
#pragma unroll
        for (int step = 32; step; step >>= 1) {
            const int cand = lo + step;
            const u32 v = (u32)wv::shfl((int)rel, cand & 63);
            if (cand < 64 && v <= t) lo = cand;
        }
        const u32 r0 = (u32)wv::shfl((int)rel, lo);
        u64 v = (u64)(u32)wv::shfl((int)xlo, lo) | ((u64)(u32)wv::shfl((int)xhi, lo) << 32);
        if (t >= total) continue;
        u32 r = t - r0, pos = 0;
#pragma unroll
        for (int sh = 32; sh; sh >>= 1) {
            const u32 c = (u32)popc64(v & ((1ULL << sh) - 1));
            if (r >= c) { r -= c; v >>= sh; pos += (u32)sh; }
        }
        npos[(u64)base + t] = (w0 + (u64)lo) * 64 + pos;
    }
}
```

autocycler_amd/csrc/kernels_tail.inc:

```
struct LinkOrderFunctor {
    const int32_t* sym; int32_t* ord; u8* cnt; u32* n_self_mirror;
    u64* n_links;
    AC_D void operator()(u64 idx, bool valid) const {
        int n = 0;
        if (valid) {
            int side = (int)(idx & 1);
            int32_t num = (int32_t)(idx >> 1) + 1;
            int32_t tmp[5]; u64 key[5];
            for (int c = 0; c < 5; c++) {
                int32_t v = sym[idx * 5 + (u64)c];
                if (v == 0) continue;
                u32 cls = (side == 0) ? (v > 0 ? 0u : 1u) : (v > 0 ? 1u : ((-v <= num) ? 0u : 2u));
                u64 kv = ((u64)cls << 32) | (u64)(v < 0 ? -v : v);
                int j = n++;
                while (j > 0 && key[j - 1] > kv) { key[j] = key[j - 1]; tmp[j] = tmp[j - 1]; j--; }
                key[j] = kv; tmp[j] = v;
            }
            u32 self = 0;
            for (int i = 0; i < 5; i++) {
                ord[idx * 5 + (u64)i] = i < n ? tmp[i] : 0;
                if (i < n && tmp[i] == (side == 0 ? -num : num)) self++;
            }
            cnt[idx] = (u8)n;
            if (self) atomic_add32(n_self_mirror, self);
// ... 685 lines not shown
    const u8* seq; u64 total; u64* words; u32* bad;
    AC_D void operator()(u64 w) const {
        const u64 b = w * 32;
        u64 x = 0; u32 wrong = 0;
        for (u32 i = 0; i < 32 && b + i < total; i++) {
            const u32 ch = seq[b + i];
            wrong += (ch != 'A' && ch != 'C' && ch != 'G' && ch != 'T') ? 1u : 0u;
            x |= (u64)(((ch >> 1) ^ (ch >> 2)) & 3u) << (2 * i);
        }
        words[w] = x;
        if (wrong) atomic_add32(bad, wrong);
    }
};
struct RemapFunctor {
    int32_t* path; const u64* number_len; const u64* path_off; u32 n_seqs; u64 n_ent; u64* sums; u64 first_wave; u32 block;
    int32_t* host_out;
    bool store;
    AC_D void operator()(u64 tid, bool valid) const {
        if (!valid) return;
        const u64 wave = first_wave + (tid >> 6);
        const u32 lane = (u32)(tid & 63);
        const u64 w0 = wave * (u64)block;
        u64 w1 = w0 + (u64)block;
        if (w1 > n_ent) w1 = n_ent;
        u32 s = 0;
        u64 acc = 0;
        u64 i = w0 + lane;
        if (i < w1) {
            u32 lo = 0, hi = n_seqs;
            while (hi - lo > 1) { u32 mid = lo + ((hi - lo) >> 1); if (path_off[mid] <= i) lo = mid; else hi = mid; }
            s = lo;
        }
        for (; i < w1; i += 64) {
            while (s + 1 < n_seqs && i >= path_off[s + 1]) { if (acc) atomic_add64(&sums[s], acc); acc = 0; s++; }
            int32_t v = path[i];
            u64 nl = number_len[idx_of(v)];
            int32_t f = (int32_t)(nl & 0xFFFFFFFFu);
            const int32_t o = v > 0 ? f : -f;
            if (store) path[i] = o;
            if (host_out) host_out[i] = o;
            acc += nl >> 32;
        }
        const u32 s0 = (u32)wv::shfl((int)s, 0);
        if (wv::all(s == s0 || acc == 0)) {
            u64 t = acc;
#pragma unroll
            for (int o = 32; o; o >>= 1) t += (u64)wv::shfl_xor64((unsigned long long)t, o);
            if (lane == 0 && t) atomic_add64(&sums[s0], t);
            return;
        }
        if (acc) atomic_add64(&sums[s], acc);
    }
};

struct SeqFunctor {
    const u64* bits; const u64* useq_off; const u64* ustartpos; const u32* ulen; const u8* uorient;
    u32 n_unitigs; u64 total; int h; u8* out; u32 per;
    AC_HD void operator()(u64 tid) const {
        const u64 g0 = tid * per;
        if (g0 >= total) return;
        u32 lo = 0, hi = n_unitigs;
        while (hi - lo > 1) { u32 mid = lo + ((hi - lo) >> 1); if (useq_off[mid] <= g0) lo = mid; else hi = mid; }
        u32 r = lo;
        for (u32 j = 0; j < per; j++) {
            const u64 g = g0 + (u64)j;
            if (g >= total) break;
            while (g >= useq_off[r] + (u64)ulen[r]) r++;
            u64 i = g - useq_off[r];
            u32 n = ulen[r];
            u32 c;
            if (uorient[r]) c = text_code(bits, ustartpos[r] + (u64)h + i);
            else c = 3u - text_code(bits, ustartpos[r] + (u64)h + ((u64)n - 1 - i));
            out[g] = (u8)("ACGT"[c]);
        }
    }
};
struct BlockMaxFunctor {
    const u64* off; u32 n_unitigs; u64 n_blocks; u32* m;
    AC_D void operator()(u64 r) const {
        const u64 b = (off[r] + 63) / 64;
        if (b < n_blocks) atomic_max32(&m[b], (u32)r);
    }
};
AC_D u8 base_char(u32 c) { return (u8)((0x54474341u >> (8 * c)) & 0xFFu); }
struct SeqSrc { const u64* bits; const u64* ustartpos; const u32* ulen; const u8* uorient; int h; };
template <int MODE>
AC_KERNEL void __launch_bounds__(256) seq_write_kernel(SeqSrc q, ExpState e, const u64* off, const u32* first, u32 n_unitigs, u64 total, u8* out) {
    AC_SHARED u32 tile[16 * 257];
    const u32 t = wv::tid();
    const u64 tid = (u64)wv::bid() * 256 + t;
    const u64 g0 = tid * 64;
    if (g0 < total) {
        u32 r = first[tid];
        u64 g = g0;
        const u64 g_end = (g0 + 64 < total) ? g0 + 64 : total;
        u32 acc = 0; int j = 0;
        while (g < g_end) {
            u64 o = off[r]; u64 o_next = (r + 1 < n_unitigs) ? off[r + 1] : total;
            while (g >= o_next) { r++; o = o_next; o_next = (r + 1 < n_unitigs) ? off[r + 1] : total; }
            const u32 i0 = (u32)(g - o);
            const u32 cnt = (u32)(((o_next < g_end) ? o_next : g_end) - g);
            if (MODE == 0) {
                const u32 n = q.ulen[r];
                const bool fwd = q.uorient[r] != 0;
                const u64 base = q.ustartpos[r] + (u64)q.h;
                for (u32 d = 0; d < cnt; d += 32) {
// ... 36 lines not shown
```

autocycler_amd/csrc/kernels_unitigs.inc:

```
template <int W> AC_D int count_successors(const TextCtx& t, const Table& tb, const XKmer<W>& x, int max_c, int known) {
    int n = 0;
    for (int c = 0; c < max_c; c++) {
        XKmer<W> y;
        if (!xk_next<W>(x, t.k, c, &y)) continue;
        if (c == known) { if (owns_xk<W>(t, tb, y)) n++; continue; }
        u64 pos; bool rel;
        if (find_xk<W>(t, tb, y, &pos, &rel)) n++;
    }
    return n;
}
template <int W> AC_D bool real_kmer_exists(const TextCtx& t, const Table& tb, const Key<W>& f, const Key<W>& r) {
    Key<W> uk = key_lt<W>(r, f) ? r : f;
    uk.w[0] |= (u64)255 << 56;
    return table_find<W>(t, tb, uk, false).found;
}
static const u32 PROBE_NOT_MINE = 0x80000000u;
template <int W> AC_D u32 probe_real_successors(const TextCtx& t, const Table& tb, const Key<W>& fwd, const Key<W>& rc, u32 want, u64* pos, u32* rel_same) {
    const int k = t.k;
    const Key<W> km = key_kmask<W>(k);
    u32 found = 0;
    if (rel_same) *rel_same = 0;
    if (k < 3) {
#pragma unroll
        for (int c = 0; c < 4; c++) {
// ... 298 lines not shown
        const Key<W>& b = sub ? fwd : rc;
        u32 cnt = 0;
        const bool mine = successor_group_is_mine<W>(tb, a, b, t.k);
        if (code) {
            const int known = sub ? (!text_mask(t.mask, p - 1) ? 3 - (int)text_code(t.bits, p - 1) : -1)
                                  : (!text_mask(t.mask, p + (u64)t.k) ? (int)text_code(t.bits, p + (u64)t.k) : -1);
            if (code >= 4u && !successor_may_branch<W>(a, b, t.k, code - 4u)) cnt = mine ? 1 : 0;
            else cnt = (u32)count_real_successors<W>(t, tb, a, b, known);
        }
        if (dot && mine) {
            const Key<W> m1 = key_kmask<W>(t.k - 1);
            Key<W> sfx = a;
AC_UNROLL_W
            for (int j = 0; j < W; j++) sfx.w[j] &= m1.w[j];
            if (endset_has<W>(es, sfx)) cnt++;
        }
        if (!cnt) return;
        atomic_add32(&kinfo[i], sub ? cnt << KI_IN_SHIFT : cnt);
    }
    AC_D void operator()(u64 tid) const {
        const int l = (int)(tid / ((u64)DEG_REGIONS * DEG_PROBE_THREADS));
        const u64 r = tid % ((u64)DEG_REGIONS * DEG_PROBE_THREADS);
        const u32 region = (u32)(r / DEG_PROBE_THREADS), j0 = (u32)(r % DEG_PROBE_THREADS);
        const u32 per = l ? 10u : 2u;
        const u64* items = wk.list(l);
        const u32 rc = wk.rcap[l];
        const u64 n = (u64)(wk.count(l)[region] < rc ? wk.count(l)[region] : rc) * per;
        for (u64 j = j0; j < n; j += DEG_PROBE_THREADS) one(l, items[(u64)region * rc + j / per], (u32)(j % per));
        const u64 no = (u64)wk.count(l)[DEG_REGIONS] * per;
        for (u64 j = r; j < no; j += (u64)DEG_REGIONS * DEG_PROBE_THREADS) one(l, items[(u64)DEG_REGIONS * rc + j / per], (u32)(j % per));
    }
};

template <int W> struct FirstFunctor {
    TextCtx t; Table tb; Novel nv; u32* kinfo; const u8* flags;
    const u32* slot; u32* words;
    AC_D void operator()(u64 s) const {
        for (int which = 0; which < 2; which++) {
            if (flags && !(flags[s] & (which ? 2u : 1u))) continue;
            u64 p = t.seq_off[s] + (which ? (u64)t.seq_len[s] - 1 : 0);
            XKmer<W> x;
            if (!xkmer_at<W>(t, p, &x)) continue;
            u64 pos; bool rel_same;
            if (!find_xk<W>(t, tb, x, &pos, &rel_same)) continue;
            u32 j = novel_rank(nv, pos);
            bool flag_on_T = (which == 0) ? rel_same : !rel_same;
            if (words) { words[slot[s] + ((which && flags && (flags[s] & 1u)) ? 1u : 0u)] = (j + 1u) | (flag_on_T ? 0u : 0x80000000u); continue; }
            atomic_or32(&kinfo[j], flag_on_T ? KI_FIRST_T : KI_FIRST_RCT);
        }
    }
};

struct HeadFunctor {
    const u64* npos; const u32* kinfo; u32* head; u64 n;
    AC_HD void operator()(u64 i) const {
        u32 h = 1;
        if (i > 0 && npos[i] == npos[i - 1] + 1) {
            u32 a = kinfo[i - 1], b = kinfo[i];
            bool internal = !(a & KI_FIRST_RCT) && (a & KI_OUT_MASK) == 1 && ((b >> KI_IN_SHIFT) & 7u) == 1 && !(b & KI_FIRST_T);
            h = internal ? 0u : 1u;
        }
        head[i] = h;
    }
};
struct UnitigStartFunctor {
    const u32* head; const u32* scan; u32* ustart; u64 n;
    AC_HD void operator()(u64 i) const { if (head[i]) ustart[scan[i] - 1] = (u32)i; }
};

template <int W> struct MinVal { Key<W> key; u32 flipped; u32 pad; };
template <int W> struct MinOp {
    AC_HD MinVal<W> operator()(const MinVal<W>& a, const MinVal<W>& b) const { return key_lt<W>(b.key, a.key) ? b : a; }
};
template <int W> struct MinValLess {
    AC_HD bool operator()(const MinVal<W>& a, const MinVal<W>& b) const { return key_lt<W>(a.key, b.key); }
};
template <int W> AC_D Key<W> canonical_at(const TextCtx& t, u64 p, bool* flipped) {
    XKmer<W> x;
    bool ok = true;
    if (text_mask_count(t.mask, p, t.k) == 0) { x.fwd = text_extract<W>(t.bits, p, t.k); x.ld = 0; x.td = 0; }
    else ok = xkmer_at<W>(t, p, &x);
    *flipped = false;
    if (ok) return xk_canonical<W>(x, t.k, flipped);
    Key<W> bad;
#pragma unroll
    for (int j = 0; j < W; j++) bad.w[j] = ~0ULL;
    return bad;
}
template <int W> struct MinIdxOp {
    TextCtx t; const u64* npos;
    AC_D u32 operator()(const u32& a, const u32& b) const {
        bool fa, fb;
        Key<W> ka = canonical_at<W>(t, npos[a], &fa), kb = canonical_at<W>(t, npos[b], &fb);
        return key_lt<W>(kb, ka) ? b : a;
    }
};
template <int W> struct CKeyFunctor {
    TextCtx t; const u64* npos; const u32* scan; MinVal<W>* vals; u32* seg;
    AC_D void operator()(u64 i) const {
        bool flipped;
        MinVal<W> v;
        v.key = canonical_at<W>(t, npos[i], &flipped);
        v.flipped = flipped ? 1u : 0u; v.pad = 0;
        vals[i] = v;
        seg[i] = scan[i] - 1;
    }
};
template <int W> struct MinWaveArgs {
    TextCtx t; const u64* npos; const u32* scan; u64 N; MinVal<W>* umin; MinVal<W>* wfirst; MinVal<W>* wlast;
};
template <int W> AC_D MinVal<W> minval_at(const MinWaveArgs<W>& a, u64 i) {
    bool flipped;
    MinVal<W> v;
    v.key = canonical_at<W>(a.t, a.npos[i], &flipped);
    v.flipped = flipped ? 1u : 0u; v.pad = 0;
    return v;
}
AC_D u64 shfl_down_u64(u64 x, int o) {
    u32 lo = (u32)wv::shfl_down((int)(u32)x, o), hi = (u32)wv::shfl_down((int)(u32)(x >> 32), o);
    return ((u64)hi << 32) | lo;
}
template <int W>
AC_KERNEL void __launch_bounds__(256) minkey_wave_kernel(MinWaveArgs<W> a) {
    const u64 i = (u64)wv::bid() * 256 + wv::tid();
    const int lane = wv::lane();
    const bool valid = i < a.N;
    const u32 seg = valid ? a.scan[i] - 1 : 0xFFFFFFFFu;
    MinVal<W> v;
    if (valid) v = minval_at<W>(a, i);
    else {
#pragma unroll
        for (int j = 0; j < W; j++) v.key.w[j] = ~0ULL;
        v.flipped = 0; v.pad = 0;
    }
    const u32 seg_prev = (u32)wv::shfl_up((int)seg, 1);
    const bool piece_start = lane == 0 || seg_prev != seg;
    const bool starts_here = valid && (i == 0 || a.scan[i - 1] - 1 != seg);
    const bool goes_on = valid && i + 1 < a.N && a.scan[i + 1] - 1 == seg;
#pragma unroll
    for (int o = 1; o < 64; o <<= 1) {
        MinVal<W> other;
#pragma unroll
        for (int j = 0; j < W; j++) other.key.w[j] = shfl_down_u64(v.key.w[j], o);
        other.flipped = (u32)wv::shfl_down((int)v.flipped, o);
        const u32 oseg = (u32)wv::shfl_down((int)seg, o);
        if (lane + o < 64 && oseg == seg && key_lt<W>(other.key, v.key)) { v.key = other.key; v.flipped = other.flipped; }
    }
    const u32 seg63 = (u32)wv::shfl((int)seg, 63);
    const int on63 = wv::shfl((int)(goes_on ? 1 : 0), 63);
    if (!valid || !piece_start) return;
    const bool reaches_end = seg == seg63;
    if (starts_here && !(reaches_end && on63)) a.umin[seg] = v;
    if (lane == 0) a.wfirst[i >> 6] = v;
    if (reaches_end) a.wlast[i >> 6] = v;
}
template <int W> struct MinJoinFunctor {
    const u32* ustart; u32 U; u64 N; const MinVal<W>* wfirst; const MinVal<W>* wlast; MinVal<W>* umin;
    AC_D void operator()(u64 u) const {
        const u64 a = ustart[u], b = (u + 1 < (u64)U ? (u64)ustart[u + 1] : N) - 1;
        const u64 wa = a >> 6, wb = b >> 6;
        if (wa == wb) return;
        MinVal<W> v = wlast[wa];
        for (u64 w = wa + 1; w <= wb; w++) {
            MinVal<W> o = wfirst[w];
            if (key_lt<W>(o.key, v.key)) v = o;
        }
        umin[u] = v;
    }
};
struct MinPre { u64 f; u32 idx; u32 tie; };
AC_HD MinPre minpre_combine(const MinPre& a, const MinPre& b) {
    if (a.f < b.f) return a;
    if (b.f < a.f) return b;
    MinPre r = a; r.tie = 1u;
    return r;
}
template <int W> AC_D MinPre minpre_at(const TextCtx& t, const u64* npos, u64 i, int max_nb) {
    const u64 p = npos[i];
    MinPre v; v.idx = (u32)i;
    if (text_mask_count(t.mask, p, t.k) != 0) { v.f = 0; v.tie = 1u; return v; }
    const int nb = t.k < max_nb ? t.k : max_nb;
    const u64 lf = text_extract<1>(t.bits, p, nb).w[0];
    const u64 lr = key_rc<1>(text_extract<1>(t.bits, p + (u64)(t.k - nb), nb), nb).w[0];
    v.f = 1 + (lf < lr ? lf : lr); v.tie = 0;
    return v;
}
struct MinPreArgs { TextCtx t; const u64* npos; const u32* scan; u64 N; MinPre* upre; MinPre* wfirst; MinPre* wlast; int max_nb; };
template <int W>
AC_KERNEL void __launch_bounds__(256) minpre_wave_kernel(MinPreArgs a) {
    const u64 i = (u64)wv::bid() * 256 + wv::tid();
    const int lane = wv::lane();
    const bool valid = i < a.N;
    const u32 seg = valid ? a.scan[i] - 1 : 0xFFFFFFFFu;
    MinPre v;
    if (valid) v = minpre_at<W>(a.t, a.npos, i, a.max_nb);
    else { v.f = ~0ULL; v.idx = 0; v.tie = 0; }
    const u32 seg_prev = (u32)wv::shfl_up((int)seg, 1);
    const bool piece_start = lane == 0 || seg_prev != seg;
    const bool starts_here = valid && (i == 0 || a.scan[i - 1] - 1 != seg);
    const bool goes_on = valid && i + 1 < a.N && a.scan[i + 1] - 1 == seg;
#pragma unroll
    for (int o = 1; o < 64; o <<= 1) {
        MinPre other;
        other.f = shfl_down_u64(v.f, o);
        other.idx = (u32)wv::shfl_down((int)v.idx, o);
        other.tie = (u32)wv::shfl_down((int)v.tie, o);
        const u32 oseg = (u32)wv::shfl_down((int)seg, o);
        if (lane + o < 64 && oseg == seg) v = minpre_combine(v, other);
    }
    const u32 seg63 = (u32)wv::shfl((int)seg, 63);
    const int on63 = wv::shfl((int)(goes_on ? 1 : 0), 63);
    if (!valid || !piece_start) return;
    const bool reaches_end = seg == seg63;
    if (starts_here && !(reaches_end && on63)) a.upre[seg] = v;
    if (lane == 0) a.wfirst[i >> 6] = v;
    if (reaches_end) a.wlast[i >> 6] = v;
}
template <int W> struct MinFinishFunctor {
    TextCtx t; const u64* npos; const u32* ustart; u32 U; u64 N; const MinPre* upre; const MinPre* wfirst; const MinPre* wlast; MinVal<W>* umin;
    AC_D void operator()(u64 u) const {
        const u64 a = ustart[u], b = (u + 1 < (u64)U ? (u64)ustart[u + 1] : N) - 1;
        const u64 wa = a >> 6, wb = b >> 6;
        MinPre v;
        if (wa == wb) v = upre[u];
        else {
            v = wlast[wa];
            for (u64 w = wa + 1; w <= wb; w++) v = minpre_combine(v, wfirst[w]);
        }
        bool flipped;
        MinVal<W> m;
        m.key = canonical_at<W>(t, npos[v.idx], &flipped);
        m.flipped = flipped ? 1u : 0u; m.pad = 0;
        if (v.tie) {
            for (u64 i = a; i <= b; i++) {
                bool fl;
                const Key<W> key = canonical_at<W>(t, npos[i], &fl);
                if (key_lt<W>(key, m.key)) { m.key = key; m.flipped = fl ? 1u : 0u; }
            }
        }
        umin[u] = m;
    }
};
template <int W> struct UnitigMinFunctor {
    TextCtx t; const u64* npos; const u32* umin_idx; MinVal<W>* umin;
    AC_D void operator()(u64 u) const {
        bool flipped;
        MinVal<W> v;
        v.key = canonical_at<W>(t, npos[umin_idx[u]], &flipped);
        v.flipped = flipped ? 1u : 0u; v.pad = 0;
        umin[u] = v;
    }
};
template <int W> struct MinValIdxLess {
// ... 12 lines not shown
    }
};
template <int W> struct SeedPrefixFunctor {
    const MinVal<W>* umin; int k; u64* key; int keep;
    u32* iota;
    AC_HD void operator()(u64 u) const {
        if (iota) iota[u] = (u32)u;
        Key<W> v = umin[u].key;
        const u64 top = v.w[0] >> 56;
        v.w[0] &= ~((u64)255 << 56);
        const int bits = 2 * k, want = top == 255 ? 63 : 55;
        u64 lead;
        if (bits >= want) lead = key_shr<W>(v, bits - want).w[W - 1];
        else lead = v.w[W - 1] << (want - bits);
        const u64 full = top == 255 ? ((1ULL << 63) | lead) : ((top << 55) | lead);
        key[u] = keep >= 64 ? full : (full >> (64 - keep)) << (64 - keep);
    }
};
template <int W> struct SeedTieFunctor {
    const u32* order; const u64* key; u64 n; const MinVal<W>* umin; u32* out; u32 max_group; u32* big;
    AC_D void operator()(u64 i) const {
        const u64 pfx = key[i];
        const u32 me = order[i];
        if ((i == 0 || key[i - 1] != pfx) && (i + 1 == n || key[i + 1] != pfx)) { out[i] = me; return; }
        u64 a = i, b = i + 1;
        while (a > 0 && key[a - 1] == pfx && b - a <= (u64)max_group) a--;
        while (b < n && key[b] == pfx && b - a <= (u64)max_group) b++;
        if (b - a > (u64)max_group) { out[i] = me; atomic_or32(big, 1u); return; }
        const Key<W> mine = umin[me].key;
        u64 r = 0;
        for (u64 j = a; j < b; j++) if (j != i && key_lt<W>(umin[order[j]].key, mine)) r++;
        out[a + r] = me;
    }
};
template <int W> struct GatherMinFunctor { const u32* order; const MinVal<W>* in; MinVal<W>* out; AC_HD void operator()(u64 r) const { out[r] = in[order[r]]; } };

template <int W> struct UnitigMetaFunctor {
    const u32* order; const u32* ustart; const u64* npos; const MinVal<W>* sorted_min; u32 n_unitigs; u64 n_novel;
    u32* rank; u32* ulen; u64* ulen64; u64* ustartpos; u8* uorient;
    AC_HD void operator()(u64 r) const {
        if (r == n_unitigs) { ulen64[r] = 0; return; }
        u32 u = order[r];
        rank[u] = (u32)r;
        u32 a = ustart[u];
        u32 b = (u + 1 < n_unitigs) ? ustart[u + 1] : (u32)n_novel;
        ulen[r] = b - a;
        ulen64[r] = (u64)(b - a);
        ustartpos[r] = npos[a];
        uorient[r] = sorted_min[r].flipped ? 0 : 1;
    }
};

struct UnitigCtx {
    const u32* head; const u32* scan; const u32* rank; const u8* uorient; const u32* ustart; const u32* ulen;
    u32 n_unitigs; u64 n_novel;
};

template <int W> struct LinksFunctor {
    TextCtx t; Table tb; Novel nv; UnitigCtx uc; const u32* order; const u64* npos; int any_dots;
    int32_t* links; u64* wlinks; u32* err;
    const V16* uinfo;
    AC_D void operator()(u64 idx) const {
        u32 r = (u32)(idx >> 1);
        int side = (int)(idx & 1);
        const V16 me = uinfo[order[r]];
        u32 ia = me.a;
        u32 ib = me.b - 1;
        bool o = (me.d & 1u) != 0;
        bool use_b = (side == 0) ? o : !o;
        XKmer<W> e;
        if (!xkmer_at<W>(t, npos[use_b ? ib : ia], &e)) { atomic_or32(err, 2u); return; }
        if (!use_b) e = xk_rc<W>(e, t.k);
        int max_c = any_dots ? 5 : 4;
        const bool grouped = e.ld == 0 && e.td == 0;
        u64 gpos[4] = {0, 0, 0, 0}; u32 grel = 0, gfound = 0;
        if (grouped) {
            Key<W> erc = key_rc<W>(e.fwd, t.k);
            gfound = probe_real_successors<W>(t, tb, e.fwd, erc, 15u, gpos, &grel);
            if (gfound == PROBE_NOT_MINE) gfound = 0;
        }
        for (int c = 0; c < 5; c++) {
            int32_t val = 0;
            u32 tlen = 0;
            XKmer<W> y;
            u64 pos = 0; bool rel_same = false;
            bool hit;
            if (grouped && c < 4) { hit = (gfound >> c) & 1u; pos = gpos[c]; rel_same = (grel >> c) & 1u; }
            else hit = c < max_c && xk_next<W>(e, t.k, c, &y) && find_xk<W>(t, tb, y, &pos, &rel_same);
            if (hit) {
                u32 j = novel_rank(nv, pos);
                const V16 tg = uinfo[uc.scan[j] - 1];
                u32 rv = tg.c;
                bool strand = rel_same ? (tg.d & 1u) != 0 : (tg.d & 1u) == 0;
                if (!(rel_same ? j == tg.a : j + 1 == tg.b)) atomic_or32(err, 4u);
                val = strand ? (int32_t)(rv + 1) : -(int32_t)(rv + 1);
                tlen = tg.b - tg.a;
            }
            links[idx * 5 + (u64)c] = val;
            wlinks[idx * 5 + (u64)c] = ((u64)tlen << 32) | (u64)(u32)val;
        }
    }
};
```

autocycler_amd/csrc/selftest_prims.inc:

```

namespace selftest {

template <class T> struct Shifted {
    DBuf<T> buf; T* p;
    Shifted(size_t n, int mis) : buf(n + 16 / sizeof(T)), p(buf.ptr() + mis) {}
};
template <class T, int OP, bool INCL> void scan_case(const void* in, u64 n, bool in_place, int mis_in, int mis_out, void* out) {
    if (mis_in < 0 || mis_out < 0 || (size_t)mis_in >= 16 / sizeof(T) || (size_t)mis_out >= 16 / sizeof(T)) throw DeviceError("selftest scan: misalignment out of range");
    Shifted<T> a(n, mis_in), o(n, mis_out);
    copy_h2d(a.p, in, n * sizeof(T));
    T* dst = in_place ? a.p : o.p;
    scan_launch<T, OP, INCL>(a.p, dst, n, 0);
    copy_d2h(out, dst, n * sizeof(T));
}

struct MinU64 { AC_HD u64 operator()(u64 a, u64 b) const { return b < a ? b : a; } };
struct ArgSmaller { const u64* v; AC_HD u32 operator()(u32 a, u32 b) const { return v[b] < v[a] ? b : a; } };
struct PairKey { u64 a; u32 b; u32 pad; };
struct PairLess { AC_HD bool operator()(const PairKey& x, const PairKey& y) const { return x.a != y.a ? x.a < y.a : x.b < y.b; } };
struct ValueLess { const u64* v; AC_HD bool operator()(u32 x, u32 y) const { return v[x] < v[y]; } };

enum WaveProgram {
    WP_BALLOT = 0, WP_ALL, WP_UNIFORM, WP_SHFL, WP_SHFL64, WP_SHFL_XOR, WP_SHFL_XOR64, WP_SHFL_UP, WP_SHFL_DOWN,
    WP_GRP_BALLOT16, WP_GRP_SHFL16, WP_GRP_BALLOT64, WP_GRP_SHFL64, WP_BLOCK_SYNC,
// ... 96 lines not shown
    if (op != 0 && op != 1) throw DeviceError("selftest segments: unknown op");
    DBuf<u32> ds(n), err(1, true); DBuf<u64> dv(n);
    copy_h2d(ds.ptr(), seg, n * 4); copy_h2d(dv.ptr(), vals, n * 8);
    u32* e = deferred_err ? err.ptr() : nullptr;
    if (op == 0) {
        DBuf<u64> o(n_segments);
        o.fill_bytes(0xFF);
        reduce_by_segment(ds.ptr(), dv.ptr(), n, o.ptr(), n_segments, selftest::MinU64(), e);
        copy_d2h(out, o.ptr(), n_segments * 8);
    } else {
        DBuf<u32> o(n_segments);
        o.fill_bytes(0xFF);
        segment_argmin(ds.ptr(), n, o.ptr(), n_segments, selftest::ArgSmaller{dv.ptr()}, e);
        copy_d2h(out, o.ptr(), n_segments * 4);
    }
    *err_out = read_scalar(err.ptr());
    stream_sync();
}

void selftest_sort_cmp(int form, const uint64_t* a, const uint32_t* b, const uint32_t* vals, uint64_t n, uint64_t* a_out, uint32_t* b_out, uint32_t* vals_out) {
    Arena::device().reset();
    if (n && (!a || !vals || !vals_out)) throw DeviceError("null pointer");
    if (n >= 0xFFFFFFF0ULL) throw DeviceError("selftest sort: too many items");
    if (form == 0) {
        if (n && (!b || !a_out || !b_out)) throw DeviceError("null pointer");
        std::vector<selftest::PairKey> hk(n);
        for (u64 i = 0; i < n; i++) hk[i] = selftest::PairKey{a[i], b[i], 0};
        DBuf<selftest::PairKey> dk(n); DBuf<u32> dv(n);
        copy_h2d(dk.ptr(), hk.data(), n * sizeof(selftest::PairKey)); copy_h2d(dv.ptr(), vals, n * 4);
        sort_by_key_cmp(dk, dv, n, selftest::PairLess());
        copy_d2h(hk.data(), dk.ptr(), n * sizeof(selftest::PairKey)); copy_d2h(vals_out, dv.ptr(), n * 4);
        for (u64 i = 0; i < n; i++) { a_out[i] = hk[i].a; b_out[i] = hk[i].b; }
    } else if (form == 1) {
        for (u64 i = 0; i < n; i++) if (vals[i] >= n) throw DeviceError("selftest sort: index out of range");
        DBuf<u64> dv(n); DBuf<u32> idx(n);
        copy_h2d(dv.ptr(), a, n * 8); copy_h2d(idx.ptr(), vals, n * 4);
        sort_keys_cmp(idx, n, selftest::ValueLess{dv.ptr()});
        copy_d2h(vals_out, idx.ptr(), n * 4);
    } else throw DeviceError("selftest sort: unknown form");
    stream_sync();
}

void selftest_scan_pool(int op, uint64_t value, uint64_t* out) {
    if (!out) throw DeviceError("null pointer");
    ScanPool& pool = scan_pool();
    if (op == 1) {
        if (value < pool.epoch || value >= (1ULL << 16)) throw DeviceError("selftest scan pool: the epoch only goes forward and stays below 2^16");
        pool.epoch = value;
    } else if (op == 2) pool.invalidate();
    else if (op != 0) throw DeviceError("selftest scan pool: unknown op");
    out[0] = pool.cap; out[1] = pool.epoch; out[2] = pool.tickets;
}

void selftest_wave(int program, const uint64_t* in_u64, const int32_t* aux_i32, const uint64_t* live_mask, uint64_t* out_u64) {
    Arena::device().reset();
    if (!in_u64 || !aux_i32 || !live_mask || !out_u64) throw DeviceError("null pointer");
    if (program < 0 || program >= selftest::WP_COUNT) throw DeviceError("selftest wave: unknown program");
    DBuf<u64> in(256), live(4), out(256); DBuf<int> aux(256);
    copy_h2d(in.ptr(), in_u64, 256 * 8); copy_h2d(aux.ptr(), aux_i32, 256 * 4); copy_h2d(live.ptr(), live_mask, 4 * 8); copy_h2d(out.ptr(), out_u64, 256 * 8);
    launch_wave_kernel(selftest::wave_program_kernel<0>, 1, 0, program, (const u64*)in.ptr(), (const int*)aux.ptr(), (const u64*)live.ptr(), out.ptr());
    copy_d2h(out_u64, out.ptr(), 256 * 8);
    stream_sync();
}
```

include/autocycler_hip.h:

```cpp
#ifndef AUTOCYCLER_HIP_H
#define AUTOCYCLER_HIP_H

#include <stddef.h>
#include <stdint.h>

#ifdef __cplusplus
extern "C" {
#endif

typedef struct ac_graph ac_graph;

typedef struct {
    const uint8_t* fwd;
    uint32_t length;
    uint16_t id;
} ac_seq_view;

typedef struct { uint32_t pos; uint16_t seq_id_and_strand; } ac_position;
typedef struct { int32_t a; int32_t b; } ac_link;
typedef struct { uint32_t unitigs; uint64_t links_one_way; uint64_t total_length; } ac_stats;

typedef struct {
    double h2d, pack, insert, collect_sort, degree, segment, minkey, rank, paths, links, seqs, d2h;
    double total_device;
// ... 22 lines not shown
    double insert_rest_known;
    double insert_rest_sampled;
    uint64_t path_stretches;
    uint32_t expand_sparse_sweeps;
    uint32_t expand_sparse_start;
} ac_timings;

int ac_compress_build(uint32_t k, uint32_t assembly_count, const ac_seq_view* seqs, uint32_t n_seqs, int device,
                      ac_graph** out);

int ac_compress_build_multi(uint32_t k, uint32_t assembly_count, const ac_seq_view* seqs, uint32_t n_seqs, const int* devices,
                            int n_devices, ac_graph** out);
typedef struct {
    uint32_t n_ranks; int transport;
    uint64_t bytes_fragments, bytes_bitmap, bytes_degrees, bytes_links, bytes_queries, bytes_answers, bytes_reduce;
    uint64_t queries_total, queries_sent_away;
    uint64_t table_capacity_max, table_capacity_sum;
    uint64_t union_text_bytes, fragments, distinct;
    double seconds_total, seconds_exchange_max;
    uint64_t candidates_total, candidates_owned_max;
    uint64_t bytes_sibling;
    uint64_t bytes_tail;
    uint64_t degrees_open;
    uint64_t bytes_received_max;
    uint64_t path_runs_copied;
} ac_multi_info;
int ac_multi_info_get(const ac_graph*, ac_multi_info* out);
size_t ac_multi_info_get_sized(const ac_graph*, ac_multi_info* out, size_t out_size);

typedef struct {
    uint32_t failed;
    uint64_t first_bad_unitig, first_bad_link, first_bad_path_entry, first_bad_sequence, first_bad_base;
    uint64_t unitigs, links, path_entries, bases_checked, self_mirror_links;
    double seconds;
    uint32_t checks;
    uint64_t first_bad_junction;
} ac_verify_report;
int ac_verify_graph(const ac_graph* graph, const ac_seq_view* seqs, uint32_t n_seqs, int device, ac_verify_report* report);
int ac_verify_graph_device(const ac_graph* graph, const void* d_text, uint64_t n_text, const uint64_t* seq_off, const uint32_t* seq_len,
                           uint32_t n_seqs, int device, ac_verify_report* report);

int ac_decompress_device(const ac_graph*, int device, uint8_t* out, uint64_t out_bytes);

int ac_selftest_primitives(int device, uint64_t n, uint64_t seed, int end_bit, int key_kind);

int ac_selftest_scan(int device, int kind, const void* in, uint64_t n, int in_place, int misalign_in, int misalign_out, void* out);
int ac_selftest_radix(int device, const uint64_t* keys, const void* vals, uint64_t n, int begin_bit, int end_bit, int val_kind, uint64_t prep_n, int prep_bits,
                      int prep_reuse, uint64_t* keys_out, void* vals_out);
int ac_selftest_segments(int device, int op, const uint32_t* seg, const uint64_t* vals, uint64_t n, uint64_t n_segments, int deferred_err, void* out, uint32_t* err_out);
int ac_selftest_sort_cmp(int device, int form, const uint64_t* key_a, const uint32_t* key_b, const uint32_t* vals, uint64_t n, uint64_t* key_a_out, uint32_t* key_b_out,
                         uint32_t* vals_out);
int ac_selftest_scan_pool(int device, int op, uint64_t value, uint64_t* out);
int ac_selftest_wave(int device, int program, const uint64_t* in_u64, const int32_t* aux_i32, const uint64_t* live_mask, uint64_t* out_u64);

int ac_selftest_fills(int device, const uint64_t* regions, uint64_t n_regions, int trigger, int mode, uint8_t* span, uint64_t span_bytes, uint32_t* launches_out);
int ac_selftest_fill_order(int device, uint64_t n, int byte1, uint64_t w_lo, uint64_t w_hi, int w_val, uint64_t from2, int byte2, uint64_t upto3, int byte3, uint8_t* out);
int ac_selftest_readback(int device, const uint8_t* data, uint64_t n_data, int path, const uint64_t* items, uint64_t n_items, uint8_t* out, uint32_t* counters_out);
int ac_selftest_scalar_chain(int device, const uint64_t* values, uint64_t n, uint64_t* out, uint32_t* counters_out);
int ac_selftest_arena(int device, const uint64_t* ops, uint64_t n_ops, uint64_t* totals_out, uint64_t* allocs_out, const uint8_t* live, uint64_t* wrong_out);
int ac_selftest_launch(int device, int which, uint64_t n, uint64_t* slots_out, uint32_t* info_out);
int ac_selftest_atomics(int device, int op, uint64_t init, uint64_t expected, const uint64_t* operand, const uint32_t* target, uint32_t n_words, uint64_t* words_out,
                        uint64_t* returns_out);
int ac_selftest_side_order(int device, int mode, int which, uint32_t seed, uint64_t n_words, uint32_t* out_words);
int ac_selftest_event_ring(int device, int op, const uint8_t* kinds, uint32_t n_more, uint64_t* out);

int ac_pack_text(const uint8_t* text, uint64_t n_text, uint64_t* bits, uint32_t* mask32, int force_scalar);

int ac_compress_build_device(uint32_t k, uint32_t assembly_count, const void* d_text, uint64_t n_text,
                             const uint64_t* seq_off, const uint32_t* seq_len, const uint16_t* seq_ids,
                             const uint16_t* seq_d1, const uint16_t* seq_d2, uint32_t n_seqs, int device,
                             ac_graph** out);

typedef struct ac_shard ac_shard;
int ac_shard_begin(uint32_t k, uint32_t local_assembly_count, const void* d_text, uint64_t n_text, const uint64_t* seq_off,
                   const uint32_t* seq_len, const uint16_t* seq_ids, const uint16_t* seq_d1, const uint16_t* seq_d2,
                   uint32_t n_seqs, int device, ac_shard** out);
int ac_shard_fragment_sizes(const ac_shard*, uint64_t* text_bytes, uint64_t* n_fragments);
int ac_shard_fragments_export(ac_shard*, void* d_text_out , void* d_meta_out );
uint64_t ac_shard_fragment_packed_words(const ac_shard*, uint64_t union_off);
int ac_shard_fragments_export_packed(ac_shard*, uint64_t union_off, void* d_words_u64, void* d_meta_out );
int ac_shard_build_union_packed(ac_shard*, uint32_t rank, uint32_t n_shards, const void* d_staged_words_u64, const uint64_t* first_word,
                                const uint64_t* n_words, uint64_t n_union_text, const void* d_meta, uint64_t n_fragments_total);
uint64_t ac_shard_local_distinct(const ac_shard*);
void ac_shard_set_distinct_upper_bound(ac_shard*, uint64_t n);
int ac_shard_build_union(ac_shard*, uint32_t rank, uint32_t n_shards, const void* d_union_text, uint64_t n_union_text,
                         const void* d_meta, uint64_t n_fragments_total);
uint64_t ac_shard_table_capacity(const ac_shard*);
uint64_t ac_shard_bitmap_words(const ac_shard*);
int ac_shard_bitmap_export(ac_shard*, void* d_out_u64);
int ac_shard_build_novel(ac_shard*, const void* d_bitmap_sum_u64 );
uint64_t ac_shard_distinct_count(const ac_shard*);
uint64_t ac_shard_sib_words(const ac_shard*);
int ac_shard_sib_export(ac_shard*, void* d_out_u64 );
int ac_shard_degrees(ac_shard*, const void* d_sib_sum_u64);
uint64_t ac_shard_degree_bytes(const ac_shard*);
int ac_shard_degrees_export(ac_shard*, void* d_out_u8 );
int ac_shard_build_graph(ac_shard*, const void* d_degrees_sum_u8 );
uint32_t ac_shard_unitig_count(const ac_shard*);
int ac_shard_links_export(ac_shard*, void* d_links_i32 , void* d_wlinks_i64 );
int ac_shard_links_import(ac_shard*, const void* d_links_sum_i32 , const void* d_wlinks_sum_i64 );
uint64_t ac_shard_query_count(const ac_shard*);
uint32_t ac_shard_query_key_words(const ac_shard*);
int ac_shard_queries_export(ac_shard*, void* d_out_u64 );
int ac_shard_answer(ac_shard*, const void* d_keys_u64, uint64_t n_queries, void* d_out_u64 );
int ac_shard_walk(ac_shard*, const void* d_answers_u64 );
int ac_shard_queries_route(ac_shard*, uint32_t n_shards, void* d_routed_keys_u64 ,
// ... 499 lines not shown
```

Measured before the change: 86660.

## Replace per-kmer head/scan arrays with head bitmap and rank-select structure

Unitig heads are now recorded as a wave-ballot bitmap with a per-word popcount prefix instead of a u32 head flag array plus an inclusive scan over all N k-mers. Segment ids are computed on the fly by rank (prefix plus masked popcount), and unitig starts come from a select pass. The novel k-mer position list is built with the same shared RankSelect helper. This cuts memory traffic and scan work over N, but adds popcount arithmetic and extra bitmap reads in several kernels. A rank-select self-test entry point is also added.

```diff
diff --git a/autocycler_amd/_capi.py b/autocycler_amd/_capi.py
--- a/autocycler_amd/_capi.py
+++ b/autocycler_amd/_capi.py
@@ -240,7 +240,7 @@
 EXPORTS = ["ac_compress_build", "ac_compress_build_multi", "ac_multi_info_get", "ac_compress_build_device", "ac_pack_text", "ac_text_size", "ac_layout_text", "ac_kmer_count",
            "ac_stats_pre", "ac_stats_post", "ac_unitig_count", "ac_unitig", "ac_unitigs_bulk", "ac_paths_bulk", "ac_unitig_positions", "ac_links",
            "ac_path", "ac_timings_get", "ac_timings_get_sized", "ac_free", "ac_gfa_string", "ac_string_free", "ac_last_error",
-           "ac_device_count", "ac_max_kmer", "ac_version", "ac_abi_version", "ac_set_host_side_device", "ac_source_hash", "ac_set_stage_timing", "ac_random_access_ceilings", "ac_random_access_ceilings_at", "ac_release_memory", "ac_end_repair_device", "ac_pairwise_distances", "ac_trim_paths", "ac_trim_path_slices", "ac_overlap_alignment", "ac_trim_max_unitigs", "ac_resolve_bridges", "ac_resolve_bridge_paths", "ac_path_distances", "ac_resolve_anchors", "ac_resolve_bridge_records", "ac_resolve_best_paths", "ac_resolve_distinct_paths", "ac_resolve_summary_get_sized", "ac_resolve_max_path", "ac_resolve_free", "ac_graph_components", "ac_components_from_links", "ac_components_records", "ac_components_of_unitig", "ac_components_members", "ac_components_unitig_flags", "ac_components_summary_get_sized", "ac_topology_name", "ac_components_free", "ac_graph_merge_plan", "ac_merge_plan_from_links", "ac_merge_chains", "ac_merge_members", "ac_merge_chain_of_unitig", "ac_merge_fixed_flags", "ac_merge_sequences", "ac_merge_links", "ac_merge_summary_get_sized", "ac_merge_free", "ac_graph_subsets", "ac_subsets_from_paths", "ac_subsets_records", "ac_subsets_unitigs", "ac_subsets_links", "ac_subsets_seqs", "ac_subsets_path_ends", "ac_subsets_dense", "ac_subsets_summary_get_sized", "ac_subsets_free", "ac_subsets_components", "ac_subsets_merge_plan", "ac_subsets_merged_paths", "ac_merged_paths_get", "ac_merged_paths_summary_get_sized", "ac_merged_paths_free", "ac_merge_finish", "ac_subsets_finish", "ac_finished_unitigs", "ac_finished_sequences", "ac_finished_new_of_old", "ac_finished_links", "ac_finished_paths", "ac_finished_summary_get_sized", "ac_finished_free", "ac_finished_gfa_string", "ac_finished_to_graph", "ac_apply_bridges", "ac_graph_resolve_apply", "ac_applied_unitigs", "ac_applied_bridge_of", "ac_applied_links", "ac_applied_bridge_sequences", "ac_applied_summary_get_sized", "ac_applied_free", "ac_applied_merge_plan", "ac_applied_finish", "ac_applied_gfa_string", "ac_resolve_graphs", "ac_clean_graph", "ac_graph_clean", "ac_cleaned_unitigs", "ac_cleaned_links", "ac_cleaned_summary_get_sized", "ac_cleaned_free", "ac_cleaned_merge_plan", "ac_cleaned_finish", "ac_cleaned_gfa_string", "ac_parse_tig_numbers", "ac_gfa_segment_types", "ac_clean_gfa", "ac_clean", "ac_trim_apply", "ac_graph_trim_apply", "ac_graph_trim", "ac_trimmed_records", "ac_trimmed_summary_get_sized", "ac_trimmed_free", "ac_trimmed_subsets", "ac_trimmed_finish", "ac_trimmed_yaml_string", "ac_trim_gfa", "ac_trim_dir", "ac_resolve_dir", "ac_cluster_tree_build", "ac_cluster_tree_from_distances", "ac_cluster_tree_from_nodes", "ac_cluster_nodes", "ac_cluster_merges", "ac_cluster_summary_get_sized", "ac_cluster_free", "ac_cluster_max_seqs", "ac_cluster_cut", "ac_cluster_assign", "ac_cluster_containment", "ac_cluster_newick", "ac_cluster_generate", "ac_cluster_qc_nodes", "ac_cluster_qc_clusters", "ac_cluster_qc_assignment", "ac_cluster_qc_records", "ac_cluster_qc_metrics", "ac_cluster_qc_trace", "ac_cluster_qc_summary_get_sized", "ac_cluster_qc_free", "ac_cluster_min_assemblies", "ac_cluster_seq_inputs", "ac_depth_begin", "ac_depth_begin_handles", "ac_depth_add_reads", "ac_depth_add_fastq", "ac_depth_totals_get", "ac_depth_kmer_counts", "ac_depth_finish", "ac_depth_free", "ac_selftest_primitives", "ac_selftest_scan", "ac_selftest_radix", "ac_selftest_segments", "ac_selftest_sort_cmp", "ac_selftest_scan_pool", "ac_selftest_wave", "ac_selftest_fills", "ac_selftest_fill_order", "ac_selftest_readback", "ac_selftest_scalar_chain", "ac_selftest_arena", "ac_selftest_launch", "ac_selftest_atomics", "ac_selftest_side_order", "ac_selftest_event_ring", "ac_verify_graph", "ac_verify_graph_device", "ac_graph_from_gfa", "ac_graph_kmer_size", "ac_graph_seq_info", "ac_decompress_seq", "ac_decompress_device", "ac_decompress",
+           "ac_device_count", "ac_max_kmer", "ac_version", "ac_abi_version", "ac_set_host_side_device", "ac_source_hash", "ac_set_stage_timing", "ac_random_access_ceilings", "ac_random_access_ceilings_at", "ac_release_memory", "ac_end_repair_device", "ac_pairwise_distances", "ac_trim_paths", "ac_trim_path_slices", "ac_overlap_alignment", "ac_trim_max_unitigs", "ac_resolve_bridges", "ac_resolve_bridge_paths", "ac_path_distances", "ac_resolve_anchors", "ac_resolve_bridge_records", "ac_resolve_best_paths", "ac_resolve_distinct_paths", "ac_resolve_summary_get_sized", "ac_resolve_max_path", "ac_resolve_free", "ac_graph_components", "ac_components_from_links", "ac_components_records", "ac_components_of_unitig", "ac_components_members", "ac_components_unitig_flags", "ac_components_summary_get_sized", "ac_topology_name", "ac_components_free", "ac_graph_merge_plan", "ac_merge_plan_from_links", "ac_merge_chains", "ac_merge_members", "ac_merge_chain_of_unitig", "ac_merge_fixed_flags", "ac_merge_sequences", "ac_merge_links", "ac_merge_summary_get_sized", "ac_merge_free", "ac_graph_subsets", "ac_subsets_from_paths", "ac_subsets_records", "ac_subsets_unitigs", "ac_subsets_links", "ac_subsets_seqs", "ac_subsets_path_ends", "ac_subsets_dense", "ac_subsets_summary_get_sized", "ac_subsets_free", "ac_subsets_components", "ac_subsets_merge_plan", "ac_subsets_merged_paths", "ac_merged_paths_get", "ac_merged_paths_summary_get_sized", "ac_merged_paths_free", "ac_merge_finish", "ac_subsets_finish", "ac_finished_unitigs", "ac_finished_sequences", "ac_finished_new_of_old", "ac_finished_links", "ac_finished_paths", "ac_finished_summary_get_sized", "ac_finished_free", "ac_finished_gfa_string", "ac_finished_to_graph", "ac_apply_bridges", "ac_graph_resolve_apply", "ac_applied_unitigs", "ac_applied_bridge_of", "ac_applied_links", "ac_applied_bridge_sequences", "ac_applied_summary_get_sized", "ac_applied_free", "ac_applied_merge_plan", "ac_applied_finish", "ac_applied_gfa_string", "ac_resolve_graphs", "ac_clean_graph", "ac_graph_clean", "ac_cleaned_unitigs", "ac_cleaned_links", "ac_cleaned_summary_get_sized", "ac_cleaned_free", "ac_cleaned_merge_plan", "ac_cleaned_finish", "ac_cleaned_gfa_string", "ac_parse_tig_numbers", "ac_gfa_segment_types", "ac_clean_gfa", "ac_clean", "ac_trim_apply", "ac_graph_trim_apply", "ac_graph_trim", "ac_trimmed_records", "ac_trimmed_summary_get_sized", "ac_trimmed_free", "ac_trimmed_subsets", "ac_trimmed_finish", "ac_trimmed_yaml_string", "ac_trim_gfa", "ac_trim_dir", "ac_resolve_dir", "ac_cluster_tree_build", "ac_cluster_tree_from_distances", "ac_cluster_tree_from_nodes", "ac_cluster_nodes", "ac_cluster_merges", "ac_cluster_summary_get_sized", "ac_cluster_free", "ac_cluster_max_seqs", "ac_cluster_cut", "ac_cluster_assign", "ac_cluster_containment", "ac_cluster_newick", "ac_cluster_generate", "ac_cluster_qc_nodes", "ac_cluster_qc_clusters", "ac_cluster_qc_assignment", "ac_cluster_qc_records", "ac_cluster_qc_metrics", "ac_cluster_qc_trace", "ac_cluster_qc_summary_get_sized", "ac_cluster_qc_free", "ac_cluster_min_assemblies", "ac_cluster_seq_inputs", "ac_depth_begin", "ac_depth_begin_handles", "ac_depth_add_reads", "ac_depth_add_fastq", "ac_depth_totals_get", "ac_depth_kmer_counts", "ac_depth_finish", "ac_depth_free", "ac_selftest_primitives", "ac_selftest_scan", "ac_selftest_radix", "ac_selftest_segments", "ac_selftest_sort_cmp", "ac_selftest_scan_pool", "ac_selftest_wave", "ac_selftest_rank_select", "ac_selftest_fills", "ac_selftest_fill_order", "ac_selftest_readback", "ac_selftest_scalar_chain", "ac_selftest_arena", "ac_selftest_launch", "ac_selftest_atomics", "ac_selftest_side_order", "ac_selftest_event_ring", "ac_verify_graph", "ac_verify_graph_device", "ac_graph_from_gfa", "ac_graph_kmer_size", "ac_graph_seq_info", "ac_decompress_seq", "ac_decompress_device", "ac_decompress",
            "ac_shard_begin", "ac_shard_fragment_sizes", "ac_shard_fragments_export", "ac_shard_build_union", "ac_shard_fragment_packed_words", "ac_shard_fragments_export_packed", "ac_shard_build_union_packed",
            "ac_shard_unitig_count", "ac_shard_table_capacity", "ac_shard_bitmap_words", "ac_shard_bitmap_export", "ac_shard_build_novel", "ac_shard_sib_words", "ac_shard_sib_export", "ac_shard_degrees",
            "ac_shard_degree_bytes", "ac_multi_info_get_sized", "ac_shard_links_export", "ac_shard_links_import",
@@ -483,7 +483,8 @@
     lib.ac_selftest_sort_cmp.argtypes = [C.c_int, C.c_int, C.c_void_p, C.c_void_p, C.c_void_p, C.c_uint64, C.c_void_p, C.c_void_p, C.c_void_p]
     lib.ac_selftest_scan_pool.argtypes = [C.c_int, C.c_int, C.c_uint64, C.POINTER(C.c_uint64)]
     lib.ac_selftest_wave.argtypes = [C.c_int, C.c_int, C.c_void_p, C.c_void_p, C.c_void_p, C.c_void_p]
-    lib.ac_selftest_fills.argtypes = [C.c_int, C.c_void_p, C.c_uint64, C.c_int, C.c_int, C.c_void_p, C.c_uint64, C.c_void_p]
+    lib.ac_selftest_rank_select.argtypes = [C.c_int, C.c_void_p, C.c_uint64, C.c_int, C.c_int, C.c_void_p, C.c_void_p, C.c_uint64, C.POINTER(C.c_uint64)]
+    lib.ac_selftest_fills.argtypes =[C.c_int, C.c_void_p, C.c_uint64, C.c_int, C.c_int, C.c_void_p, C.c_uint64, C.c_void_p]
     lib.ac_selftest_fill_order.argtypes = [C.c_int, C.c_uint64, C.c_int, C.c_uint64, C.c_uint64, C.c_int, C.c_uint64, C.c_int, C.c_uint64, C.c_int, C.c_void_p]
     lib.ac_selftest_readback.argtypes = [C.c_int, C.c_void_p, C.c_uint64, C.c_int, C.c_void_p, C.c_uint64, C.c_void_p, C.c_void_p]
     lib.ac_selftest_scalar_chain.argtypes = [C.c_int, C.c_void_p, C.c_uint64, C.c_void_p, C.c_void_p]
@@ -2066,6 +2067,23 @@
     return out
 
 
+RANK_SELECT_POS = {None: 0, "u32": 1, "u64": 2}
+
+
+def selftest_rank_select(words, pos=None, misalign=0, pos_cap=None, device=0, lib_path=None):
+    import numpy as np
+    lib = load_library(lib_path)
+    w = _np_in(words, np.uint64)
+    if pos_cap is None:
+        pos_cap = 64 * w.size
+    prefix = np.empty(w.size + 1, dtype=np.uint32)
+    out = np.empty(pos_cap, dtype=np.uint32 if pos == "u32" else np.uint64) if pos else None
+    total = C.c_uint64()
+    _check(lib, lib.ac_selftest_rank_select(device, w.ctypes.data, w.size, misalign, RANK_SELECT_POS[pos], prefix.ctypes.data,
+                                            out.ctypes.data if pos else None, pos_cap if pos else 0, C.byref(total)))
+    return prefix, (out[:total.value] if pos else None), total.value
+
+
 FILL_KINDS = {"all": 0, "from": 1, "first": 2, "side_stream": 3}
 FILL_TRIGGERS = {"none": 0, "launch": 1, "launch_full": 2, "launch_wave_kernel": 3, "copy_h2d": 4, "copy_d2h": 5, "copy_d2d": 6, "stream_sync": 7,
                  "arena_rewind": 8, "after_main": 9, "main_event": 10}
diff --git a/autocycler_amd/csrc/capi_steps.cpp b/autocycler_amd/csrc/capi_steps.cpp
--- a/autocycler_amd/csrc/capi_steps.cpp
+++ b/autocycler_amd/csrc/capi_steps.cpp
@@ -1793,6 +1793,10 @@
 int ac_selftest_wave(int device, int program, const uint64_t* in_u64, const int32_t* aux_i32, const uint64_t* live_mask, uint64_t* out_u64) {
     return guarded([&] { DeviceCall call(device); selftest_wave(program, in_u64, aux_i32, live_mask, out_u64); });
 }
+int ac_selftest_rank_select(int device, const uint64_t* words, uint64_t n_words, int misalign, int pos_kind, uint32_t* prefix_out, void* pos_out, uint64_t pos_cap,
+                            uint64_t* total_out) {
+    return guarded([&] { DeviceCall call(device); selftest_rank_select(words, n_words, misalign, pos_kind, prefix_out, pos_out, pos_cap, total_out); });
+}
 int ac_selftest_fills(int device, const uint64_t* regions, uint64_t n_regions, int trigger, int mode, uint8_t* span, uint64_t span_bytes, uint32_t* launches_out) {
     return guarded([&] { DeviceCall call(device); selftest_fills(regions, n_regions, trigger, mode, span, span_bytes, launches_out); });
 }
diff --git a/autocycler_amd/csrc/graph_build.hpp b/autocycler_amd/csrc/graph_build.hpp
--- a/autocycler_amd/csrc/graph_build.hpp
+++ b/autocycler_amd/csrc/graph_build.hpp
@@ -201,6 +201,7 @@
 void selftest_sort_cmp(int form, const uint64_t* a, const uint32_t* b, const uint32_t* vals, uint64_t n, uint64_t* a_out, uint32_t* b_out, uint32_t* vals_out);
 void selftest_scan_pool(int op, uint64_t value, uint64_t* out);
 void selftest_wave(int program, const uint64_t* in_u64, const int32_t* aux_i32, const uint64_t* live_mask, uint64_t* out_u64);
+void selftest_rank_select(const uint64_t* words, uint64_t n_words, int misalign, int pos_kind, uint32_t* prefix_out, void* pos_out, uint64_t pos_cap, uint64_t* total_out);
 void selftest_fills(const uint64_t* regions, uint64_t n_regions, int trigger, int mode, uint8_t* span, uint64_t span_bytes, uint32_t* launches_out);
 void selftest_fill_order(uint64_t n, int byte1, uint64_t w_lo, uint64_t w_hi, int w_val, uint64_t from2, int byte2, uint64_t upto3, int byte3, uint8_t* out);
 void selftest_readback(const uint8_t* data, uint64_t n_data, int path, const uint64_t* items, uint64_t n_items, uint8_t* out, uint32_t* counters_out);
diff --git a/autocycler_amd/csrc/graph_impl.hpp b/autocycler_amd/csrc/graph_impl.hpp
--- a/autocycler_amd/csrc/graph_impl.hpp
+++ b/autocycler_amd/csrc/graph_impl.hpp
@@ -500,7 +500,7 @@
     DBuf<u64> slots; u64 cap = 0; u64 N = 0;
     DBuf<u64> bm; DBuf<u32> wprefix; DBuf<u64> npos;
     u32 U = 0;
-    DBuf<u32> kinfo, head, scan, ustart, order, rank, ulen;
+    DBuf<u32> kinfo, hprefix, ustart, order, rank, ulen; DBuf<u64> hbm;
     DBuf<u64> ustartpos, useq_off; DBuf<u8> uorient;
     DBuf<int32_t> links; DBuf<u64> wlinks;
     DBuf<u32> depth, minpos_fwd, minpos_rev; DBuf<u64> path_off; DBuf<int32_t> ent_val; u64 n_ent = 0;
@@ -620,21 +620,24 @@
 inline void GraphBuilder::Impl::novel_list(u64 known_n) {
     PackedText& g = *G;
     u64 n_bm_words = g.n_text / 64 + 1;
-    DBuf<u32> wcnt(n_bm_words + 1);
+    RankSelect rs;
     wprefix.alloc(n_bm_words + 1);
-    launch(n_bm_words + 1, PopcFunctor{bm.ptr(), wcnt.ptr(), n_bm_words});
-    exclusive_scan_u32(wcnt.ptr(), wprefix.ptr(), n_bm_words + 1);
+    rs.count(bm.ptr(), n_bm_words);
     if (known_n) N = known_n;
     else {
-        N = read_scalar(wprefix.ptr() + n_bm_words);
+        N = read_scalar(rs.total_ptr());
         if (N == 0) throw DeviceError("internal error: no k-mers in the union of the shards");
         tm->n_distinct = N;
     }
     npos.alloc(N);
-    launch_wave_kernel(fill_novel_wave_kernel<0>, (n_bm_words + 255) / 256, 0, (const u64*)bm.ptr(), (const u32*)wprefix.ptr(), npos.ptr(), n_bm_words);
+    rs.select<u64>(wprefix.ptr(), npos.ptr());
     kinfo.alloc(N, true);
-    head.alloc(N + 1); scan.alloc(N + 1);
-    head.fill_bytes_from(N * 4, 0); scan.fill_bytes_from(N * 4, 0);
+    hbm.alloc(N / 64 + 1); hprefix.alloc(N / 64 + 2);
+#ifdef AC_EMU
+    hbm.fill_bytes(0);
+#else
+    hbm.fill_bytes_from((N / 64) * 8, 0);
+#endif
     lap(&tm->collect_sort);
 }
 
diff --git a/autocycler_amd/csrc/graph_stages.hip b/autocycler_amd/csrc/graph_stages.hip
--- a/autocycler_amd/csrc/graph_stages.hip
+++ b/autocycler_amd/csrc/graph_stages.hip
@@ -345,15 +345,17 @@
     TextCtx t = g.ctx((int)k);
     Table tb = graph_table();
     Novel nv{bm.ptr(), wprefix.ptr()};
-    launch(N, HeadFunctor{npos.ptr(), kinfo.ptr(), head.ptr(), N});
-    inclusive_scan_u32(head.ptr(), scan.ptr(), N);
-    U = read_scalar(scan.ptr() + (N - 1));
+    launch_full(N, HeadFunctor{npos.ptr(), kinfo.ptr(), hbm.ptr(), N});
+    RankSelect heads;
+    heads.count(hbm.ptr(), N / 64 + 1);
+    U = read_scalar(heads.total_ptr());
+    const HeadRank hr{hbm.ptr(), hprefix.ptr()};
     ustart.alloc((u64)U + 1);
     int seed_keep = seed_prefix_bits();
     if (seed_keep <= 0) { int lg = 1; while ((1ULL << lg) < (u64)U) lg++; seed_keep = std::min(64, ((2 * lg + 8 + 7) / 8) * 8); }
     RadixScratch seed_rs; DBuf<u32> seed_big(1, true);
     if (seed_prefix_sort()) seed_rs.prepare(U, seed_keep);
-    launch(N, UnitigStartFunctor{head.ptr(), scan.ptr(), ustart.ptr(), N});
+    heads.select<u32>(hprefix.ptr(), ustart.ptr());
     lap(&tm->segment);
 
     DBuf<MinVal<W>> umin(U);
@@ -361,24 +363,26 @@
     if (mk == 2) {
         const u64 n_waves = (N + 63) / 64;
         DBuf<MinPre> upre(U), wfirst(n_waves), wlast(n_waves);
-        MinPreArgs a{t, npos.ptr(), scan.ptr(), N, upre.ptr(), wfirst.ptr(), wlast.ptr(), minkey_prefix_bases()};
+        MinPreArgs a{t, npos.ptr(), hr, N, upre.ptr(), wfirst.ptr(), wlast.ptr(), minkey_prefix_bases()};
         launch_wave_kernel(minpre_wave_kernel<W>, (N + 255) / 256, 0, a);
         launch(U, MinFinishFunctor<W>{t, npos.ptr(), ustart.ptr(), U, N, upre.ptr(), wfirst.ptr(), wlast.ptr(), umin.ptr()});
     } else if constexpr (W <= 4) {
         if (mk == 1) {
             const u64 n_waves = (N + 63) / 64;
             DBuf<MinVal<W>> wfirst(n_waves), wlast(n_waves);
-            MinWaveArgs<W> a{t, npos.ptr(), scan.ptr(), N, umin.ptr(), wfirst.ptr(), wlast.ptr()};
+            MinWaveArgs<W> a{t, npos.ptr(), hr, N, umin.ptr(), wfirst.ptr(), wlast.ptr()};
             launch_wave_kernel(minkey_wave_kernel<W>, (N + 255) / 256, 0, a);
             launch(U, MinJoinFunctor<W>{ustart.ptr(), U, N, wfirst.ptr(), wlast.ptr(), umin.ptr()});
         } else {
             DBuf<MinVal<W>> vals(N); DBuf<u32> seg(N);
-            launch(N, CKeyFunctor<W>{t, npos.ptr(), scan.ptr(), vals.ptr(), seg.ptr()});
+            launch(N, CKeyFunctor<W>{t, npos.ptr(), hr, vals.ptr(), seg.ptr()});
             reduce_by_segment(seg.ptr(), vals.ptr(), N, umin.ptr(), U, MinOp<W>(), counters.ptr() + 3);
         }
     } else {
         DBuf<u32> umin_idx(U);
-        segment_argmin(scan.ptr(), N, umin_idx.ptr(), U, MinIdxOp<W>{t, npos.ptr()}, counters.ptr() + 3);
+        DBuf<u32> seg(N);
+        launch(N, HeadSegFunctor{hr, seg.ptr()});
+        segment_argmin(seg.ptr(), N, umin_idx.ptr(), U, MinIdxOp<W>{t, npos.ptr()}, counters.ptr() + 3);
         launch(U, UnitigMinFunctor<W>{t, npos.ptr(), umin_idx.ptr(), umin.ptr()});
     }
     lap(&tm->minkey);
@@ -428,7 +432,7 @@
     launch((u64)U + 1, UnitigMetaFunctor<W>{order.ptr(), ustart.ptr(), npos.ptr(), umin.ptr(), U, N, rank.ptr(), ulen.ptr(),
                                             ulen64.ptr(), ustartpos.ptr(), uorient.ptr()});
     exclusive_scan_u64(ulen64.ptr(), useq_off.ptr(), (u64)U + 1);
-    UnitigCtx uc{head.ptr(), scan.ptr(), rank.ptr(), uorient.ptr(), ustart.ptr(), ulen.ptr(), U, N};
+    UnitigCtx uc{HeadRank{hbm.ptr(), hprefix.ptr()}, rank.ptr(), uorient.ptr(), ustart.ptr(), ulen.ptr(), U, N};
     lap(&tm->rank);
 
     links.alloc((u64)U * 10); wlinks.alloc((u64)U * 10);
@@ -444,10 +448,8 @@
     cplan = CopyPlan();
     if (run_rows && loc_bm.size() && PC <= 65535) {
         const u64 nw = loc.n_text / 64 + 1;
-        DBuf<u32> wcnt(nw + 1);
         loc_wprefix.alloc(nw + 1);
-        launch(nw + 1, PopcFunctor{loc_bm.ptr(), wcnt.ptr(), nw});
-        exclusive_scan_u32(wcnt.ptr(), loc_wprefix.ptr(), nw + 1);
+        rank_only(loc_bm.ptr(), nw, loc_wprefix.ptr());
         if (walk_copy_prepare<W>(PC, Novel{loc_bm.ptr(), loc_wprefix.ptr()})) n_walkers = cplan.NW;
     }
     n_queries = n_walkers + loc.n_seqs;
@@ -517,7 +519,7 @@
     TextCtx t = loc.ctx((int)k), g = G->ctx((int)k);
     Table tb = graph_table();
     Novel nv{bm.ptr(), wprefix.ptr()};
-    UnitigCtx uc{head.ptr(), scan.ptr(), rank.ptr(), uorient.ptr(), ustart.ptr(), ulen.ptr(), U, N};
+    UnitigCtx uc{HeadRank{hbm.ptr(), hprefix.ptr()}, rank.ptr(), uorient.ptr(), ustart.ptr(), ulen.ptr(), U, N};
     CopyPlan& c = cplan;
     const u64 R = c.R, NW = c.NW;
     DBuf<u64> wcount(NW + 1), woff(NW + 1);
@@ -568,7 +570,7 @@
     TextCtx t = loc.ctx((int)k), g = G->ctx((int)k);
     Table tb = graph_table();
     Novel nv{bm.ptr(), wprefix.ptr()};
-    UnitigCtx uc{head.ptr(), scan.ptr(), rank.ptr(), uorient.ptr(), ustart.ptr(), ulen.ptr(), U, N};
+    UnitigCtx uc{HeadRank{hbm.ptr(), hprefix.ptr()}, rank.ptr(), uorient.ptr(), ustart.ptr(), ulen.ptr(), U, N};
     const u32 PC = path_chunk(N, U);
     u64 n_walkers = (loc.n_text + PC - 1) / PC;
     pos_cap_now = (exact_positions || walk_answers || n_owners > 1 || G != &loc || pos_cap() == 0) ? 0xFFFFFFFFu : pos_cap();
diff --git a/autocycler_amd/csrc/graph_tail.hip b/autocycler_amd/csrc/graph_tail.hip
--- a/autocycler_amd/csrc/graph_tail.hip
+++ b/autocycler_amd/csrc/graph_tail.hip
@@ -483,7 +483,10 @@
             const u64 RB = remap_block();
             const u64 n_waves = (n_ent + RB - 1) / RB;
             const u64 w_split = host_stretch ? std::min<u64>(stretch_split_wave, n_waves) : n_waves;
-            if (w_split) launch_full(w_split * 64, RemapFunctor{m.ent_val.ptr(), number_len_text.ptr(), m.path_off.ptr(), n_seqs, n_ent, sums.ptr(), 0, (u32)RB, nullptr, false});
+            if (w_split) {
+                const u64 end = std::min<u64>(w_split * RB, n_ent), SB = std::min<u64>(RB, 1024);
+                launch_full((end + SB - 1) / SB * 64, RemapSumFunctor{m.ent_val.ptr(), number_len_text.ptr(), m.path_off.ptr(), n_seqs, end, sums.ptr(), (u32)SB});
+            }
             if (w_split < n_waves) {
                 const u64 n_chunks = 4, per_chunk = std::max<u64>((n_waves - w_split + n_chunks - 1) / n_chunks, 64);
                 for (u64 w = w_split; w < n_waves; w += per_chunk) {
diff --git a/autocycler_amd/csrc/kernels_paths.inc b/autocycler_amd/csrc/kernels_paths.inc
--- a/autocycler_amd/csrc/kernels_paths.inc
+++ b/autocycler_amd/csrc/kernels_paths.inc
@@ -145,7 +145,7 @@
                 rel_same = (((a >> 62) & 1) != 0) == flipped;
             } else if (!find_xk<W>(g, tb, x, &pos, &rel_same)) { atomic_or32(err, 8u); break; }
             u32 jn = novel_rank(nv, pos);
-            u32 r = uc.scan[jn] - 1;
+            u32 r = head_rank(uc.hr, jn) - 1;
             const V16 ui = uinfo[r];
             const u32 a = ui.a, b = ui.b;
             bool strand = rel_same;
diff --git a/autocycler_amd/csrc/kernels_table.inc b/autocycler_amd/csrc/kernels_table.inc
--- a/autocycler_amd/csrc/kernels_table.inc
+++ b/autocycler_amd/csrc/kernels_table.inc
@@ -224,22 +224,34 @@
         if (fl) atomic_or64(&sib[p >> 5], fl << (2 * (p & 31)));
     }
 };
-struct PopcFunctor {
-    const u64* bm; u32* cnt; u64 n;
-    AC_HD void operator()(u64 w) const { cnt[w] = w < n ? (u32)popc64(bm[w]) : 0u; }
-};
-template <int UNUSED> AC_KERNEL void __launch_bounds__(256) fill_novel_wave_kernel(const u64* bm, const u32* wprefix, u64* npos, u64 n_words) {
+template <int UNUSED> AC_KERNEL void __launch_bounds__(256) rank_group_count_kernel(const u64* bm, u64 n_words, u32* gcnt, u64 n_groups) {
+    const u64 w = (u64)wv::bid() * 256 + wv::tid();
+    const u64 g = w >> 6;
+    if (g > n_groups) return;
+    u32 c = w < n_words ? (u32)popc64(bm[w]) : 0u;
+#pragma unroll
+    for (int o = 32; o; o >>= 1) c += (u32)wv::shfl_xor((int)c, o);
+    if (wv::lane() == 0) gcnt[g] = c;
+}
+template <class P> AC_KERNEL void __launch_bounds__(256) rank_select_wave_kernel(const u64* bm, const u32* gprefix, u32* word_prefix, P* out, u64 n_words) {
     const u64 w = (u64)wv::bid() * 256 + wv::tid();
     const int lane = wv::lane();
     const u64 w0 = w - (u64)lane;
     if (w0 >= n_words) return;
-    const u64 x = w < n_words ? bm[w] : 0;
-    const u32 start = w < n_words ? wprefix[w] : 0;
+    const bool valid = w < n_words;
+    const u64 x = valid ? bm[w] : 0;
     const u32 cnt = (u32)popc64(x);
-    const u32 base = (u32)wv::shfl((int)start, 0);
-    const u32 rel = w < n_words ? start - base : 0xFFFFFFFFu;
-    const u64 lastv = n_words - w0 - 1;
-    const u32 total = (u32)wv::shfl((int)(rel + cnt), lastv > 63 ? 63 : (int)lastv);
+    const u32 base = gprefix[w0 >> 6];
+    u32 incl = cnt;
+#pragma unroll
+    for (int o = 1; o < 64; o <<= 1) { const u32 up = (u32)wv::shfl_up((int)incl, o); if (lane >= o) incl += up; }
+    const u32 total = (u32)wv::shfl((int)incl, 63);
+    if (valid) {
+        word_prefix[w] = base + incl - cnt;
+        if (w == n_words - 1) word_prefix[n_words] = base + incl;
+    }
+    if (!out) return;
+    const u32 rel = valid ? incl - cnt : 0xFFFFFFFFu;
     const u32 xlo = (u32)x, xhi = (u32)(x >> 32);
     for (u32 t0 = 0; t0 < total; t0 += 64) {
         const u32 t = t0 + (u32)lane;
@@ -259,6 +271,22 @@
             const u32 c = (u32)popc64(v & ((1ULL << sh) - 1));
             if (r >= c) { r -= c; v >>= sh; pos += (u32)sh; }
         }
-        npos[(u64)base + t] = (w0 + (u64)lo) * 64 + pos;
-    }
-}
+        out[(u64)base + t] = (P)((w0 + (u64)lo) * 64 + pos);
+    }
+}
+struct RankSelect {
+    const u64* bm = nullptr; u64 n_words = 0, n_groups = 0;
+    DBuf<u32> gprefix;
+    void count(const u64* words, u64 nw) {
+        if (nw == 0) throw DeviceError("rank_select: empty bitmap");
+        bm = words; n_words = nw; n_groups = nw / 64 + 1;
+        gprefix.alloc(n_groups + 1);
+        launch_wave_kernel(rank_group_count_kernel<0>, ((n_groups + 1) * 64 + 255) / 256, 0, bm, n_words, gprefix.ptr(), n_groups);
+        exclusive_scan_u32(gprefix.ptr(), gprefix.ptr(), n_groups + 1);
+    }
+    const u32* total_ptr() const { return gprefix.ptr() + n_groups; }
+    template <class P> void select(u32* word_prefix, P* out) {
+        launch_wave_kernel(rank_select_wave_kernel<P>, (n_words + 255) / 256, 0, bm, (const u32*)gprefix.ptr(), word_prefix, out, n_words);
+    }
+};
+inline void rank_only(const u64* words, u64 n_words, u32* word_prefix) { RankSelect rs; rs.count(words, n_words); rs.select<u32>(word_prefix, nullptr); }
diff --git a/autocycler_amd/csrc/kernels_tail.inc b/autocycler_amd/csrc/kernels_tail.inc
--- a/autocycler_amd/csrc/kernels_tail.inc
+++ b/autocycler_amd/csrc/kernels_tail.inc
@@ -761,6 +761,48 @@
         if (acc) atomic_add64(&sums[s], acc);
     }
 };
+struct RemapSumFunctor {
+    const int32_t* path; const u64* number_len; const u64* path_off; u32 n_seqs; u64 end; u64* sums; u32 block;
+    AC_D void operator()(u64 tid, bool valid) const {
+        if (!valid) return;
+        const u32 lane = (u32)(tid & 63);
+        const u64 w0 = (tid >> 6) * (u64)block;
+        u64 w1 = w0 + (u64)block;
+        if (w1 > end) w1 = end;
+        u32 s = 0;
+        u64 acc = 0, next = ~0ULL;
+        u64 i = w0 + lane;
+        if (i < w1) {
+            u32 lo = 0, hi = n_seqs;
+            while (hi - lo > 1) { u32 mid = lo + ((hi - lo) >> 1); if (path_off[mid] <= i) lo = mid; else hi = mid; }
+            s = lo;
+            if (s + 1 < n_seqs) next = path_off[s + 1];
+        }
+        auto add = [&](u64 at, u64 nl) {
+            while (at >= next) { if (acc) atomic_add64(&sums[s], acc); acc = 0; s++; next = s + 1 < n_seqs ? path_off[s + 1] : ~0ULL; }
+            acc += nl >> 32;
+        };
+        for (; i + 192 < w1; i += 256) {
+            int32_t v[4]; u64 nl[4];
+#pragma unroll
+            for (int q = 0; q < 4; q++) v[q] = path[i + 64 * (u64)q];
+#pragma unroll
+            for (int q = 0; q < 4; q++) nl[q] = number_len[idx_of(v[q])];
+#pragma unroll
+            for (int q = 0; q < 4; q++) add(i + 64 * (u64)q, nl[q]);
+        }
+        for (; i < w1; i += 64) add(i, number_len[idx_of(path[i])]);
+        const u32 s0 = (u32)wv::shfl((int)s, 0);
+        if (wv::all(s == s0 || acc == 0)) {
+            u64 t = acc;
+#pragma unroll
+            for (int o = 32; o; o >>= 1) t += (u64)wv::shfl_xor64((unsigned long long)t, o);
+            if (lane == 0 && t) atomic_add64(&sums[s0], t);
+            return;
+        }
+        if (acc) atomic_add64(&sums[s], acc);
+    }
+};
 
 struct SeqFunctor {
     const u64* bits; const u64* useq_off; const u64* ustartpos; const u32* ulen; const u8* uorient;
diff --git a/autocycler_amd/csrc/kernels_unitigs.inc b/autocycler_amd/csrc/kernels_unitigs.inc
--- a/autocycler_amd/csrc/kernels_unitigs.inc
+++ b/autocycler_amd/csrc/kernels_unitigs.inc
@@ -374,21 +374,44 @@
 };
 
 struct HeadFunctor {
-    const u64* npos; const u32* kinfo; u32* head; u64 n;
-    AC_HD void operator()(u64 i) const {
-        u32 h = 1;
-        if (i > 0 && npos[i] == npos[i - 1] + 1) {
+    const u64* npos; const u32* kinfo; u64* hbm; u64 n;
+    AC_D void operator()(u64 i, bool valid) const {
+        bool h = valid;
+        if (valid && i > 0 && npos[i] == npos[i - 1] + 1) {
             u32 a = kinfo[i - 1], b = kinfo[i];
             bool internal = !(a & KI_FIRST_RCT) && (a & KI_OUT_MASK) == 1 && ((b >> KI_IN_SHIFT) & 7u) == 1 && !(b & KI_FIRST_T);
-            h = internal ? 0u : 1u;
-        }
-        head[i] = h;
-    }
-};
-struct UnitigStartFunctor {
-    const u32* head; const u32* scan; u32* ustart; u64 n;
-    AC_HD void operator()(u64 i) const { if (head[i]) ustart[scan[i] - 1] = (u32)i; }
-};
+            h = !internal;
+        }
+        const u64 word = wv::ballot(h);
+        if ((i & 63) == 0 && valid) hbm[i >> 6] = word;
+    }
+};
+struct HeadRank {
+    const u64* hbm;
+    const u32* hprefix;
+};
+AC_HD u32 head_rank(const HeadRank& hr, u64 i) {
+    const u64 w = i >> 6;
+    return hr.hprefix[w] + (u32)popc64(hr.hbm[w] & (~0ULL >> (63 - (int)(i & 63))));
+}
+struct HeadSegFunctor {
+    HeadRank hr; u32* seg;
+    AC_HD void operator()(u64 i) const { seg[i] = head_rank(hr, i) - 1; }
+};
+struct HeadLane { u32 seg; bool starts_here, goes_on; };
+AC_D HeadLane head_lane(const HeadRank& hr, u64 i, int lane, bool valid, u64 N) {
+    const u64 w = i >> 6;
+    const bool wave_in = i - (u64)lane < N;
+    const u64 word = wave_in ? hr.hbm[w] : 0;
+    const u32 base = wave_in ? hr.hprefix[w] : 0;
+    HeadLane r;
+    r.seg = valid ? base + (u32)popc64(word & (~0ULL >> (63 - lane))) - 1 : 0xFFFFFFFFu;
+    r.starts_here = valid && ((word >> lane) & 1);
+    bool next_head = true;
+    if (valid && i + 1 < N) next_head = ((lane < 63 ? word >> (lane + 1) : hr.hbm[w + 1]) & 1) != 0;
+    r.goes_on = valid && i + 1 < N && !next_head;
+    return r;
+}
 
 template <int W> struct MinVal { Key<W> key; u32 flipped; u32 pad; };
 template <int W> struct MinOp {
@@ -418,18 +441,18 @@
     }
 };
 template <int W> struct CKeyFunctor {
-    TextCtx t; const u64* npos; const u32* scan; MinVal<W>* vals; u32* seg;
+    TextCtx t; const u64* npos; HeadRank hr; MinVal<W>* vals; u32* seg;
     AC_D void operator()(u64 i) const {
         bool flipped;
         MinVal<W> v;
         v.key = canonical_at<W>(t, npos[i], &flipped);
         v.flipped = flipped ? 1u : 0u; v.pad = 0;
         vals[i] = v;
-        seg[i] = scan[i] - 1;
+        seg[i] = head_rank(hr, i) - 1;
     }
 };
 template <int W> struct MinWaveArgs {
-    TextCtx t; const u64* npos; const u32* scan; u64 N; MinVal<W>* umin; MinVal<W>* wfirst; MinVal<W>* wlast;
+    TextCtx t; const u64* npos; HeadRank hr; u64 N; MinVal<W>* umin; MinVal<W>* wfirst; MinVal<W>* wlast;
 };
 template <int W> AC_D MinVal<W> minval_at(const MinWaveArgs<W>& a, u64 i) {
     bool flipped;
@@ -447,7 +470,8 @@
     const u64 i = (u64)wv::bid() * 256 + wv::tid();
     const int lane = wv::lane();
     const bool valid = i < a.N;
-    const u32 seg = valid ? a.scan[i] - 1 : 0xFFFFFFFFu;
+    const HeadLane hl = head_lane(a.hr, i, lane, valid, a.N);
+    const u32 seg = hl.seg;
     MinVal<W> v;
     if (valid) v = minval_at<W>(a, i);
     else {
@@ -457,8 +481,7 @@
     }
     const u32 seg_prev = (u32)wv::shfl_up((int)seg, 1);
     const bool piece_start = lane == 0 || seg_prev != seg;
-    const bool starts_here = valid && (i == 0 || a.scan[i - 1] - 1 != seg);
-    const bool goes_on = valid && i + 1 < a.N && a.scan[i + 1] - 1 == seg;
+    const bool starts_here = hl.starts_here, goes_on = hl.goes_on;
 #pragma unroll
     for (int o = 1; o < 64; o <<= 1) {
         MinVal<W> other;
@@ -507,20 +530,20 @@
     v.f = 1 + (lf < lr ? lf : lr); v.tie = 0;
     return v;
 }
-struct MinPreArgs { TextCtx t; const u64* npos; const u32* scan; u64 N; MinPre* upre; MinPre* wfirst; MinPre* wlast; int max_nb; };
+struct MinPreArgs { TextCtx t; const u64* npos; HeadRank hr; u64 N; MinPre* upre; MinPre* wfirst; MinPre* wlast; int max_nb; };
 template <int W>
 AC_KERNEL void __launch_bounds__(256) minpre_wave_kernel(MinPreArgs a) {
     const u64 i = (u64)wv::bid() * 256 + wv::tid();
     const int lane = wv::lane();
     const bool valid = i < a.N;
-    const u32 seg = valid ? a.scan[i] - 1 : 0xFFFFFFFFu;
+    const HeadLane hl = head_lane(a.hr, i, lane, valid, a.N);
+    const u32 seg = hl.seg;
     MinPre v;
     if (valid) v = minpre_at<W>(a.t, a.npos, i, a.max_nb);
     else { v.f = ~0ULL; v.idx = 0; v.tie = 0; }
     const u32 seg_prev = (u32)wv::shfl_up((int)seg, 1);
     const bool piece_start = lane == 0 || seg_prev != seg;
-    const bool starts_here = valid && (i == 0 || a.scan[i - 1] - 1 != seg);
-    const bool goes_on = valid && i + 1 < a.N && a.scan[i + 1] - 1 == seg;
+    const bool starts_here = hl.starts_here, goes_on = hl.goes_on;
 #pragma unroll
     for (int o = 1; o < 64; o <<= 1) {
         MinPre other;
@@ -639,7 +662,7 @@
 };
 
 struct UnitigCtx {
-    const u32* head; const u32* scan; const u32* rank; const u8* uorient; const u32* ustart; const u32* ulen;
+    HeadRank hr; const u32* rank; const u8* uorient; const u32* ustart; const u32* ulen;
     u32 n_unitigs; u64 n_novel;
 };
 
@@ -676,7 +699,7 @@
             else hit = c < max_c && xk_next<W>(e, t.k, c, &y) && find_xk<W>(t, tb, y, &pos, &rel_same);
             if (hit) {
                 u32 j = novel_rank(nv, pos);
-                const V16 tg = uinfo[uc.scan[j] - 1];
+                const V16 tg = uinfo[head_rank(uc.hr, j) - 1];
                 u32 rv = tg.c;
                 bool strand = rel_same ? (tg.d & 1u) != 0 : (tg.d & 1u) == 0;
                 if (!(rel_same ? j == tg.a : j + 1 == tg.b)) atomic_or32(err, 4u);
diff --git a/autocycler_amd/csrc/selftest_prims.inc b/autocycler_amd/csrc/selftest_prims.inc
--- a/autocycler_amd/csrc/selftest_prims.inc
+++ b/autocycler_amd/csrc/selftest_prims.inc
@@ -172,6 +172,33 @@
     out[0] = pool.cap; out[1] = pool.epoch; out[2] = pool.tickets;
 }
 
+void selftest_rank_select(const uint64_t* words, uint64_t n_words, int misalign, int pos_kind, uint32_t* prefix_out, void* pos_out, uint64_t pos_cap, uint64_t* total_out) {
+    Arena::device().reset();
+    if (!words || !prefix_out || !total_out || (pos_kind && pos_cap && !pos_out)) throw DeviceError("null pointer");
+    if (n_words == 0 || n_words >= (1ULL << 26)) throw DeviceError("selftest rank_select: word count out of range");
+    if (misalign < 0 || misalign > 1) throw DeviceError("selftest rank_select: misalignment out of range");
+    if (pos_kind < 0 || pos_kind > 2) throw DeviceError("selftest rank_select: unknown position kind");
+    selftest::Shifted<u64> bm(n_words, misalign);
+    copy_h2d(bm.p, words, n_words * 8);
+    DBuf<u32> prefix(n_words + 1);
+    RankSelect rs;
+    rs.count(bm.p, n_words);
+    const u64 total = read_scalar(rs.total_ptr());
+    *total_out = total;
+    if (pos_kind && total > pos_cap) throw DeviceError("selftest rank_select: " + std::to_string(total) + " set bits, room for " + std::to_string(pos_cap));
+    if (pos_kind == 1) {
+        DBuf<u32> pos(total);
+        rs.select<u32>(prefix.ptr(), pos.ptr());
+        copy_d2h(pos_out, pos.ptr(), total * 4);
+    } else if (pos_kind == 2) {
+        DBuf<u64> pos(total);
+        rs.select<u64>(prefix.ptr(), pos.ptr());
+        copy_d2h(pos_out, pos.ptr(), total * 8);
+    } else rs.select<u32>(prefix.ptr(), nullptr);
+    copy_d2h(prefix_out, prefix.ptr(), (n_words + 1) * 4);
+    stream_sync();
+}
+
 void selftest_wave(int program, const uint64_t* in_u64, const int32_t* aux_i32, const uint64_t* live_mask, uint64_t* out_u64) {
     Arena::device().reset();
     if (!in_u64 || !aux_i32 || !live_mask || !out_u64) throw DeviceError("null pointer");
diff --git a/include/autocycler_hip.h b/include/autocycler_hip.h
--- a/include/autocycler_hip.h
+++ b/include/autocycler_hip.h
@@ -98,6 +98,8 @@
                          uint32_t* vals_out);
 int ac_selftest_scan_pool(int device, int op, uint64_t value, uint64_t* out);
 int ac_selftest_wave(int device, int program, const uint64_t* in_u64, const int32_t* aux_i32, const uint64_t* live_mask, uint64_t* out_u64);
+int ac_selftest_rank_select(int device, const uint64_t* words, uint64_t n_words, int misalign, int pos_kind, uint32_t* prefix_out, void* pos_out, uint64_t pos_cap,
+                            uint64_t* total_out);
 
 int ac_selftest_fills(int device, const uint64_t* regions, uint64_t n_regions, int trigger, int mode, uint8_t* span, uint64_t span_bytes, uint32_t* launches_out);
 int ac_selftest_fill_order(int device, uint64_t n, int byte1, uint64_t w_lo, uint64_t w_hi, int w_val, uint64_t from2, int byte2, uint64_t upto3, int byte3, uint8_t* out);
```

Result: no change. 86000 (-0.8%).
